# LuizGuzzo/Monocular_Depth_Estimation

Hardware: AMD Instinct MI355X
Metric: training images/sec at 640x480 bs=32/GPU (GuideDepth, SSIM+0.1*L1, Adam) (higher is better)
Workload: dtype fp32; 1 GPU; GuideDepth (DDRNet-23-slim + 3 guided upsampling blocks) train step, BASELINE cfg2, BN in train mode; global_batch=32, per_gpu_batch=32, resolution=640x480, parallelism=dp1

## Files before the change

### include/mde_abi.h

```cpp
#ifndef MDE_ABI_H
#define MDE_ABI_H

#include <stddef.h>
#include <stdint.h>

#ifdef __cplusplus
extern "C" {
#endif

#define MDE_ABI_VERSION 1

#define MDE_F32 0
#define MDE_BF16 1

#define MDE_OK 0
#define MDE_ERR_INVALID_ARG (-1)
#define MDE_ERR_UNSUPPORTED (-2)

int mde_abi_version(void);
const char* mde_status_string(int status);


int mde_bilinear_fwd(const void* x, void* y, int64_t n, int64_t c, int64_t hi,
                     int64_t wi, int64_t ho, int64_t wo, float scale_h,
                     float scale_w, int align_corners, int dtype, void* stream);
int mde_bilinear_bwd(const void* gy, void* gx, int64_t n, int64_t c,
                     int64_t hi, int64_t wi, int64_t ho, int64_t wo,
                     float scale_h, float scale_w, int align_corners,
                     int dtype, void* stream);
int mde_bilinear_bwd2_supported(int64_t n, int64_t c, int64_t hi, int64_t wi, int64_t ho,
                                int64_t wo, float scale_h, float scale_w, int align_corners);
int mde_bilinear_bwd2(const void* gy, const void* gy2, void* gx, int64_t n, int64_t c,
                      int64_t hi, int64_t wi, int64_t ho, int64_t wo, float scale_h,
                      float scale_w, int align_corners, int dtype, void* stream);

int mde_nearest_fwd(const void* x, void* y, int64_t n, int64_t c, int64_t hi,
                    int64_t wi, int64_t ho, int64_t wo, float scale_h,
                    float scale_w, int dtype, void* stream);
int mde_nearest_bwd(const void* gy, void* gx, int64_t n, int64_t c, int64_t hi,
                    int64_t wi, int64_t ho, int64_t wo, float scale_h,
                    float scale_w, int dtype, void* stream);
int mde_nearest_pyramid_supported(int64_t n, int64_t c, int64_t h, int64_t w);
int mde_nearest_pyramid(const void* x, void* half, void* quarter, int64_t n, int64_t c, int64_t h,
                        int64_t w, int dtype, void* stream);

size_t mde_se_workspace(int64_t n, int64_t c, int64_t cr, int64_t h,
                        int64_t w);
int mde_se_fwd(const void* xa, int64_t ca, const void* xb, int64_t cb,
               const float* w1, const float* w2, int64_t cr, void* out,
               float* s, float* hidden, float* mean, int64_t n, int64_t h,
               int64_t w, void* workspace, int dtype, void* stream);
int mde_se_bwd(const void* gout, const void* xa, int64_t ca, const void* xb,
               int64_t cb, const float* w1, const float* w2, int64_t cr,
               const float* s, const float* hidden, const float* mean,
               void* gxa, void* gxb, float* gw1, float* gw2, int64_t n,
               int64_t h, int64_t w, void* workspace, int dtype, void* stream);
int mde_se_gate_fwd(const void* xa, int64_t ca, const void* xb, int64_t cb,
                    const float* w1, const float* b1, const float* w2, const float* b2,
                    int64_t cr, int gate, void* out, float* s, float* hidden, float* mean,
                    int64_t n, int64_t h, int64_t w, void* workspace, int dtype,
                    void* stream);
int mde_se_gate_bwd(const void* gout, const void* xa, int64_t ca, const void* xb,
                    int64_t cb, const float* w1, const float* w2, const float* b2,
                    int64_t cr, int gate, const float* s, const float* hidden,
                    const float* mean, void* gxa, void* gxb, float* gw1, float* gb1,
                    float* gw2, float* gb2, int64_t n, int64_t h, int64_t w,
                    void* workspace, int dtype, void* stream);
size_t mde_se_bn_workspace(int64_t n, int64_t c, int64_t cr, int64_t h, int64_t w);
int mde_se_bn_fwd(const void* ya, int64_t ca, const void* yb, int64_t cb, const float* scale,
                  const float* shift, const float* w1, const float* w2, int64_t cr, void* out,
                  float* s, float* hidden, float* mean, int64_t n, int64_t h, int64_t w,
                  void* workspace, int dtype, void* stream);
int mde_se_bn_bwd(const void* gout, const void* ya, int64_t ca, const void* yb, int64_t cb,
                  const float* scale, const float* shift, const float* bn_mean,
                  const float* bn_invstd, int training, const float* w1, const float* w2,
                  int64_t cr, const float* s, const float* hidden, const float* mean, void* gya,
                  void* gyb, float* ggamma, float* gbeta, float* gw1, float* gw2, int64_t n,
                  int64_t h, int64_t w, void* workspace, int dtype, void* stream);

int mde_skip_reduce_fwd(const void* r, const void* d, const float* wt,
                        const float* b, void* out, int64_t n, int64_t cin,
                        int64_t cout, int64_t h, int64_t w, int dtype,
                        void* stream);
size_t mde_skip_reduce_workspace(int64_t n, int64_t cin, int64_t cout,
                                 int64_t h, int64_t w);
int mde_skip_reduce_bwd(const void* gout, const void* r, const void* d,
                        const float* wt, void* gs, float* gw, float* gb,
                        int64_t n, int64_t cin, int64_t cout, int64_t h,
                        int64_t w, void* workspace, int dtype, void* stream);
int mde_skip_reduce_bn_supported(int64_t cin, int64_t cout, int64_t h, int64_t w, int sums);
size_t mde_skip_reduce_bn_workspace(int64_t n, int64_t cin, int64_t cout, int64_t h, int64_t w);
int mde_skip_reduce_bn_fwd(const void* r, const void* d, const float* in_scale,
                           const float* in_shift, const float* wt, const float* b, void* out,
                           int64_t n, int64_t cin, int64_t cout, int64_t h, int64_t w, int dtype,
                           void* stream);
int mde_skip_reduce_bn_bwd(const void* gout, const void* r, const void* d, const float* in_scale,
                           const float* in_shift, const float* in_mean, const float* wt, void* gs,
                           float* gw, float* gb, float* in_sums, int64_t n, int64_t cin,
                           int64_t cout, int64_t h, int64_t w, void* workspace, int dtype,
                           void* stream);

size_t mde_minmax_workspace(int64_t numel);
int mde_minmax(const void* x, int64_t numel, float* minmax, void* workspace,
               int dtype, void* stream);
int mde_depthnorm_apply(const void* x, const float* minmax, void* y,
                        int64_t numel, int dtype, void* stream);

size_t mde_ssim3_l1_workspace(int64_t b, int64_t h, int64_t w);
int mde_ssim3_l1_fwd(const void* pred, const void* target,
                     const float* target_minmax, float w_ssim, float w_l1,
                     float* loss, void* grad_pred, void* grad_target,
                     int64_t b, int64_t h, int64_t w, void* workspace,
                     int dtype, void* stream);

size_t mde_depth_loss_workspace(int64_t b, int64_t h, int64_t w);
int mde_depth_loss_fwd(const void* pred, const void* gt, float alpha,
                       float beta, float gamma, float max_depth, float* out,
                       int64_t b, int64_t h, int64_t w, void* workspace,
                       int dtype, void* stream);
int mde_depth_loss_bwd(const void* pred, const void* gt, float alpha,
                       float beta, float gamma, float max_depth,
                       const float* fwd_out, const float* gout,
                       void* grad_pred, int64_t b, int64_t h, int64_t w,
                       void* workspace, int dtype, void* stream);

size_t mde_batchnorm_workspace(int64_t n, int64_t c, int64_t h, int64_t w);
int mde_batchnorm_fwd_train(const void* x, const float* gamma, const float* beta,
                            const float* prebias, float* running_mean,
                            float* running_var, int64_t* num_batches_tracked,
                            float momentum, float eps, const void* residual,
                            void* y, float* save_mean, float* save_invstd,
                            int64_t n, int64_t c, int64_t h, int64_t w, int act,
                            void* workspace, int dtype, void* stream);
int mde_batchnorm_fwd_eval(const void* x, const float* gamma, const float* beta,
                           const float* prebias, const float* running_mean,
                           const float* running_var, float eps,
                           const void* residual, void* y, float* save_mean,
                           float* save_invstd, int64_t n, int64_t c, int64_t h,
                           int64_t w, int act, int dtype, void* stream);
int mde_batchnorm_fwd_coef(const void* x, const float* gamma, const float* beta,
                           const float* prebias, float* running_mean, float* running_var,
                           int64_t* num_batches_tracked, float momentum, float eps,
                           int training, float* scale, float* shift, float* save_mean,
                           float* save_invstd, int64_t n, int64_t c, int64_t h, int64_t w,
                           void* workspace, int dtype, void* stream);
int mde_batchnorm_bwd(const void* gy, const void* x, const void* residual,
                      const float* gamma, const float* beta, const float* mean,
                      const float* invstd, int training, void* gx,
                      void* gresidual, float* ggamma, float* gbeta,
                      float* gprebias, int64_t n, int64_t c, int64_t h,
                      int64_t w, int act, void* workspace, int dtype,
                      void* stream);
int mde_batchnorm_fwd_train_stats(const void* x, const float* gamma, const float* beta,
                                  const float* prebias, float* running_mean, float* running_var,
                                  int64_t* num_batches_tracked, float momentum, float eps,
                                  const void* residual, void* y, float* save_mean,
                                  float* save_invstd, int64_t n, int64_t c, int64_t h, int64_t w,
                                  int act, const float* stats, int64_t stats_blocks,
                                  void* workspace, int dtype, void* stream);
int mde_batchnorm_fwd_coef_stats(const void* x, const float* gamma, const float* beta,
                                 const float* prebias, float* running_mean, float* running_var,
                                 int64_t* num_batches_tracked, float momentum, float eps,
                                 float* scale, float* shift, float* save_mean, float* save_invstd,
                                 int64_t n, int64_t c, int64_t h, int64_t w, const float* stats,
                                 int64_t stats_blocks, void* workspace, int dtype, void* stream);
int mde_batchnorm_bwd_apply(const void* gy, const void* x, const void* residual,
                            const float* gamma, const float* beta, const float* mean,
                            const float* invstd, int training, const float* sums, void* gx,
                            void* gresidual, float* ggamma, float* gbeta, float* gprebias,
                            int64_t n, int64_t c, int64_t h, int64_t w, int act, int dtype,
                            void* stream);

size_t mde_window_attn_workspace(int64_t b, int64_t h, int64_t w, int64_t c,
                                 int64_t heads, int64_t window);
int mde_window_attn_fwd(const void* qk, const float* qk_bias, const void* v,
                        const float* v_bias, const float* table, void* out, int64_t b,
                        int64_t h, int64_t w, int64_t c, int64_t heads, int64_t window,
                        int64_t shift, int dtype, void* stream);
int mde_window_attn_bwd(const void* gout, const void* qk, const float* qk_bias,
                        const void* v, const float* v_bias, const float* table, void* gqk,
                        void* gv, float* gtable, float* gqk_bias, float* gv_bias, int64_t b,
                        int64_t h, int64_t w, int64_t c, int64_t heads, int64_t window,
                        int64_t shift, void* workspace, int dtype, void* stream);

size_t mde_colsum_workspace(int64_t t_rows, int64_t n);
int mde_colsum(const void* g, float* gb, int64_t t_rows, int64_t n, void* workspace, int dtype,
               void* stream);
int mde_gelu_bwd_colsum(const void* dh, const void* a, void* da, float* gb, int64_t t_rows,
                        int64_t n, void* workspace, int dtype, void* stream);

size_t mde_linear_wgrad_workspace(int64_t t_rows, int64_t m, int64_t n);
int mde_linear_wgrad(const void* g, const void* x, float* gw, float* gb, int64_t t_rows,
                     int64_t m, int64_t n, void* workspace, int dtype, void* stream);

size_t mde_chansum_workspace(int64_t n, int64_t c, int64_t hw);
int mde_chansum(const void* g, float* gb, int64_t n, int64_t c, int64_t hw, void* workspace,
                int dtype, void* stream);

int mde_head_conv_supported(int64_t n, int64_t c, int64_t h, int64_t w);
int mde_head_conv_fwd(const void* x, const float* weight, const float* bias, void* y, int64_t n,
                      int64_t c, int64_t h, int64_t w, int dtype, void* stream);
int mde_head_conv_dgrad(const void* gy, const float* weight, void* gx, int64_t n, int64_t c,
                        int64_t h, int64_t w, int dtype, void* stream);
size_t mde_head_conv_wgrad_workspace(int64_t n, int64_t c, int64_t h, int64_t w);
int mde_head_conv_wgrad(const void* gy, const void* x, float* gweight, int64_t n, int64_t c,
                        int64_t h, int64_t w, void* workspace, int dtype, void* stream);

int mde_pointwise_supported(int64_t cin, int64_t cout, int64_t h, int64_t w);
size_t mde_pointwise_workspace(int64_t n, int64_t cin, int64_t cout, int64_t h, int64_t w);
int mde_pointwise_fwd(const void* x, const float* in_scale, const float* in_shift,
                      const float* weight, void* y, int64_t n, int64_t cin, int64_t cout,
                      int64_t h, int64_t w, int dtype, void* stream);
int mde_pointwise_bwd(const void* gy, const void* x, const float* in_scale,
                      const float* in_shift, const float* weight, void* gx, float* gweight,
                      int64_t n, int64_t cin, int64_t cout, int64_t h, int64_t w,
                      void* workspace, int dtype, void* stream);
int mde_pointwise_stats_blocks(int64_t n, int64_t cin, int64_t cout, int64_t h, int64_t w);
int mde_pointwise_fwd_stats(const void* x, const float* in_scale, const float* in_shift,
                            const float* weight, void* y, float* stats, int64_t n, int64_t cin,
                            int64_t cout, int64_t h, int64_t w, int dtype, void* stream);
int mde_pointwise_bwd_bn(const void* gy, const void* x, const float* in_scale,
                         const float* in_shift, const float* in_mean, const float* weight,
                         void* gx, float* gweight, float* in_sums, int64_t n, int64_t cin,
                         int64_t cout, int64_t h, int64_t w, void* workspace, int dtype,
                         void* stream);

int mde_conv3x3_supported(int64_t cin, int64_t cout, int pass, int dtype);
int mde_conv3x3_fwd(const void* x, const float* weight, void* y, int64_t n, int64_t cin,
                    int64_t cout, int64_t h, int64_t w, int dtype, void* stream);
int mde_conv3x3_stats_blocks(int64_t n, int64_t cin, int64_t cout, int64_t h, int64_t w,
                             int dtype);
int mde_conv3x3_fwd_stats(const void* x, const float* weight, void* y, float* stats, int64_t n,
                          int64_t cin, int64_t cout, int64_t h, int64_t w, int dtype,
                          void* stream);
int mde_conv3x3_bwd_data(const void* gy, const float* weight, void* gx, int64_t n,
                         int64_t cin, int64_t cout, int64_t h, int64_t w, int dtype,
                         void* stream);
size_t mde_conv3x3_wgrad_workspace(int64_t n, int64_t cin, int64_t cout, int64_t h, int64_t w,
                                   int dtype);
int mde_conv3x3_wgrad(const void* gy, const void* x, float* gweight, int64_t n, int64_t cin,
                      int64_t cout, int64_t h, int64_t w, void* workspace, int dtype,
                      void* stream);

int mde_conv3x3s2_supported(int64_t cin, int64_t cout, int dtype);
size_t mde_conv3x3s2_wgrad_workspace(int64_t n, int64_t cin, int64_t cout, int64_t h, int64_t w,
                                     int dtype);
int mde_conv3x3s2_wgrad(const void* gy, const void* x, float* gweight, int64_t n, int64_t cin,
                        int64_t cout, int64_t h, int64_t w, void* workspace, int dtype,
                        void* stream);

size_t mde_dwconv_workspace(int64_t n, int64_t c, int64_t h, int64_t w, int64_t k,
                            int64_t stride, int64_t pad);
int mde_dwconv_fwd(const void* x, const float* weight, void* y, int64_t n, int64_t c,
                   int64_t h, int64_t w, int64_t k, int64_t stride, int64_t pad, int dtype,
                   void* stream);
int mde_dwconv_bwd(const void* gy, const void* x, const float* weight, void* gx,
                   float* gweight, int64_t n, int64_t c, int64_t h, int64_t w, int64_t k,
                   int64_t stride, int64_t pad, void* workspace, int dtype, void* stream);

size_t mde_layernorm_workspace(int64_t rows, int64_t c);
int mde_layernorm_fwd(const void* x, const float* gamma, const float* beta, void* y,
                      float* mean, float* rstd, int64_t rows, int64_t c, float eps, int dtype,
                      void* stream);
int mde_layernorm_bwd(const void* gy, const void* x, const float* gamma, const float* mean,
                      const float* rstd, void* gx, float* ggamma, float* gbeta, int64_t rows,
                      int64_t c, void* workspace, int dtype, void* stream);
int mde_layernorm_add_fwd(const void* x, const void* r, const float* gamma, const float* beta,
                          void* sum, void* y, float* mean, float* rstd, int64_t rows, int64_t c,
                          float eps, int dtype, void* stream);
int mde_layernorm_bwd_res(const void* gy, const void* x, const void* gres, const float* gamma,
                          const float* mean, const float* rstd, void* gx, float* ggamma,
                          float* gbeta, int64_t rows, int64_t c, void* workspace, int dtype,
                          void* stream);

int mde_transpose(const void* x, void* y, int64_t batch, int64_t m, int64_t n, int dtype,
                  void* stream);

int mde_nyu_augment(const void* image, const void* depth, const int32_t* flags, float* image_out,
                    float* depth_out, int64_t n, int64_t h, int64_t w, int64_t dh, int64_t dw,
                    int depth_bits, void* stream);

size_t mde_eval_workspace(int64_t n, int64_t h, int64_t w);
int mde_eval_sums(const void* pred, const void* gt, int64_t n, int64_t h, int64_t w,
                  float min_depth, float max_depth, int mode, const int32_t* crop,
                  void* workspace, double* sums, int dtype, void* stream);

int mde_conv3x3_guide_bf16_stats_blocks(int64_t n, int64_t cout, int64_t h, int64_t w);
int mde_conv3x3_guide_bf16_fwd(const float* x, const float* weight, void* y, float* stats,
                               int64_t n, int64_t cout, int64_t h, int64_t w, void* stream);

int mde_conv1x1_supported(int64_t cin, int64_t cout, int64_t h, int64_t w, int stride,
                          int dtype);
int mde_conv1x1_fwd(const void* x, const float* weight, void* y, int64_t n, int64_t cin,
                    int64_t cout, int64_t h, int64_t w, int stride, int dtype, void* stream);
int mde_conv1x1_bwd_data(const void* gy, const float* weight, void* gx, int64_t n, int64_t cin,
                         int64_t cout, int64_t h, int64_t w, int stride, int dtype,
                         void* stream);
size_t mde_conv1x1_wgrad_workspace(int64_t n, int64_t cin, int64_t cout, int64_t h, int64_t w,
                                   int stride, int dtype);
int mde_conv1x1_wgrad(const void* gy, const void* x, float* gweight, int64_t n, int64_t cin,
                      int64_t cout, int64_t h, int64_t w, int stride, void* workspace, int dtype,
                      void* stream);

int mde_conv3x3s2_fwd_supported(int64_t cin, int64_t cout, int64_t h, int64_t w, int dtype);
int mde_conv3x3s2_dgrad_supported(int64_t cin, int64_t cout, int64_t h, int64_t w, int dtype);
int mde_conv3x3s2_fwd(const void* x, const float* weight, void* y, int64_t n, int64_t cin,
                      int64_t cout, int64_t h, int64_t w, int dtype, void* stream);
int mde_conv3x3s2_bwd_data(const void* gy, const float* weight, void* gx, int64_t n, int64_t cin,
// ... 93 lines not shown
```

### monocular_depth_estimation_amd/_abi.py

```python
from __future__ import annotations

import ctypes
import os

import torch

LIB_PATH = os.environ.get("MDE_HIP_LIB") or os.path.join(
    os.path.dirname(os.path.abspath(__file__)), "libmde_hip.so")

MDE_F32 = 0
MDE_BF16 = 1

_c = ctypes
_vp = _c.c_void_p
_i64 = _c.c_int64
_f32 = _c.c_float
_int = _c.c_int
_sz = _c.c_size_t
_fp = _c.POINTER(_c.c_float)

SIGNATURES = {
    "mde_abi_version": (_int, []),
    "mde_status_string": (_c.c_char_p, [_int]),
    "mde_bilinear_fwd": (_int, [_vp, _vp, _i64, _i64, _i64, _i64, _i64, _i64, _f32, _f32, _int, _int, _vp]),
    "mde_bilinear_bwd": (_int, [_vp, _vp, _i64, _i64, _i64, _i64, _i64, _i64, _f32, _f32, _int, _int, _vp]),
    "mde_bilinear_bwd2_supported": (_int, [_i64, _i64, _i64, _i64, _i64, _i64, _f32, _f32, _int]),
    "mde_bilinear_bwd2": (_int, [_vp, _vp, _vp, _i64, _i64, _i64, _i64, _i64, _i64, _f32, _f32, _int,
                                 _int, _vp]),
    "mde_nearest_fwd": (_int, [_vp, _vp, _i64, _i64, _i64, _i64, _i64, _i64, _f32, _f32, _int, _vp]),
    "mde_nearest_bwd": (_int, [_vp, _vp, _i64, _i64, _i64, _i64, _i64, _i64, _f32, _f32, _int, _vp]),
    "mde_nearest_pyramid_supported": (_int, [_i64, _i64, _i64, _i64]),
    "mde_nearest_pyramid": (_int, [_vp, _vp, _vp, _i64, _i64, _i64, _i64, _int, _vp]),
    "mde_se_workspace": (_sz, [_i64, _i64, _i64, _i64, _i64]),
    "mde_se_fwd": (_int, [_vp, _i64, _vp, _i64, _vp, _vp, _i64, _vp, _vp, _vp, _vp,
                          _i64, _i64, _i64, _vp, _int, _vp]),
    "mde_se_bwd": (_int, [_vp, _vp, _i64, _vp, _i64, _vp, _vp, _i64, _vp, _vp, _vp,
                          _vp, _vp, _vp, _vp, _i64, _i64, _i64, _vp, _int, _vp]),
    "mde_se_bn_workspace": (_sz, [_i64, _i64, _i64, _i64, _i64]),
    "mde_se_bn_fwd": (_int, [_vp, _i64, _vp, _i64, _vp, _vp, _vp, _vp, _i64, _vp, _vp, _vp, _vp,
                             _i64, _i64, _i64, _vp, _int, _vp]),
    "mde_se_bn_bwd": (_int, [_vp, _vp, _i64, _vp, _i64, _vp, _vp, _vp, _vp, _int, _vp, _vp, _i64,
                             _vp, _vp, _vp, _vp, _vp, _vp, _vp, _vp, _vp, _i64, _i64, _i64, _vp,
                             _int, _vp]),
    "mde_skip_reduce_fwd": (_int, [_vp, _vp, _vp, _vp, _vp, _i64, _i64, _i64, _i64, _i64, _int, _vp]),
    "mde_skip_reduce_workspace": (_sz, [_i64, _i64, _i64, _i64, _i64]),
    "mde_skip_reduce_bwd": (_int, [_vp, _vp, _vp, _vp, _vp, _vp, _vp, _i64, _i64, _i64, _i64, _i64,
                                   _vp, _int, _vp]),
    "mde_skip_reduce_bn_supported": (_int, [_i64, _i64, _i64, _i64, _int]),
    "mde_skip_reduce_bn_workspace": (_sz, [_i64, _i64, _i64, _i64, _i64]),
    "mde_skip_reduce_bn_fwd": (_int, [_vp, _vp, _vp, _vp, _vp, _vp, _vp, _i64, _i64, _i64, _i64, _i64,
                                      _int, _vp]),
    "mde_skip_reduce_bn_bwd": (_int, [_vp, _vp, _vp, _vp, _vp, _vp, _vp, _vp, _vp, _vp, _vp, _i64,
                                      _i64, _i64, _i64, _i64, _vp, _int, _vp]),
    "mde_minmax_workspace": (_sz, [_i64]),
    "mde_minmax": (_int, [_vp, _i64, _vp, _vp, _int, _vp]),
    "mde_depthnorm_apply": (_int, [_vp, _vp, _vp, _i64, _int, _vp]),
    "mde_ssim3_l1_workspace": (_sz, [_i64, _i64, _i64]),
    "mde_ssim3_l1_fwd": (_int, [_vp, _vp, _vp, _f32, _f32, _vp, _vp, _vp, _i64, _i64, _i64, _vp, _int, _vp]),
    "mde_depth_loss_workspace": (_sz, [_i64, _i64, _i64]),
    "mde_depth_loss_fwd": (_int, [_vp, _vp, _f32, _f32, _f32, _f32, _vp, _i64, _i64, _i64, _vp, _int, _vp]),
    "mde_depth_loss_bwd": (_int, [_vp, _vp, _f32, _f32, _f32, _f32, _vp, _vp, _vp, _i64, _i64, _i64,
                                  _vp, _int, _vp]),
    "mde_batchnorm_workspace": (_sz, [_i64, _i64, _i64, _i64]),
    "mde_batchnorm_fwd_train": (_int, [_vp, _vp, _vp, _vp, _vp, _vp, _vp, _f32, _f32, _vp, _vp, _vp,
                                       _vp, _i64, _i64, _i64, _i64, _int, _vp, _int, _vp]),
    "mde_batchnorm_fwd_eval": (_int, [_vp, _vp, _vp, _vp, _vp, _vp, _f32, _vp, _vp, _vp, _vp,
                                      _i64, _i64, _i64, _i64, _int, _int, _vp]),
    "mde_batchnorm_bwd": (_int, [_vp, _vp, _vp, _vp, _vp, _vp, _vp, _int, _vp, _vp, _vp, _vp, _vp,
                                 _i64, _i64, _i64, _i64, _int, _vp, _int, _vp]),
    "mde_batchnorm_bwd_apply": (_int, [_vp, _vp, _vp, _vp, _vp, _vp, _vp, _int, _vp, _vp, _vp, _vp,
                                       _vp, _vp, _i64, _i64, _i64, _i64, _int, _int, _vp]),
    "mde_window_attn_workspace": (_sz, [_i64, _i64, _i64, _i64, _i64, _i64]),
    "mde_window_attn_fwd": (_int, [_vp, _vp, _vp, _vp, _vp, _vp, _i64, _i64, _i64, _i64, _i64, _i64,
                                   _i64, _int, _vp]),
    "mde_window_attn_bwd": (_int, [_vp, _vp, _vp, _vp, _vp, _vp, _vp, _vp, _vp, _vp, _vp, _i64, _i64,
                                   _i64, _i64, _i64, _i64, _i64, _vp, _int, _vp]),
    "mde_se_gate_fwd": (_int, [_vp, _i64, _vp, _i64, _vp, _vp, _vp, _vp, _i64, _int, _vp, _vp, _vp,
                               _vp, _i64, _i64, _i64, _vp, _int, _vp]),
    "mde_se_gate_bwd": (_int, [_vp, _vp, _i64, _vp, _i64, _vp, _vp, _vp, _i64, _int, _vp, _vp, _vp,
                               _vp, _vp, _vp, _vp, _vp, _vp, _i64, _i64, _i64, _vp, _int, _vp]),
    "mde_pointwise_supported": (_int, [_i64, _i64, _i64, _i64]),
    "mde_pointwise_workspace": (_sz, [_i64, _i64, _i64, _i64, _i64]),
    "mde_pointwise_fwd": (_int, [_vp, _vp, _vp, _vp, _vp, _i64, _i64, _i64, _i64, _i64, _int, _vp]),
    "mde_pointwise_bwd": (_int, [_vp, _vp, _vp, _vp, _vp, _vp, _vp, _i64, _i64, _i64, _i64, _i64,
                                 _vp, _int, _vp]),
    "mde_pointwise_stats_blocks": (_int, [_i64, _i64, _i64, _i64, _i64]),
    "mde_pointwise_fwd_stats": (_int, [_vp, _vp, _vp, _vp, _vp, _vp, _i64, _i64, _i64, _i64, _i64,
                                       _int, _vp]),
    "mde_conv3x3_stats_blocks": (_int, [_i64, _i64, _i64, _i64, _i64, _int]),
    "mde_conv3x3_fwd_stats": (_int, [_vp, _vp, _vp, _vp, _i64, _i64, _i64, _i64, _i64, _int, _vp]),
    "mde_batchnorm_fwd_train_stats": (_int, [_vp, _vp, _vp, _vp, _vp, _vp, _vp, _f32, _f32, _vp,
                                             _vp, _vp, _vp, _i64, _i64, _i64, _i64, _int, _vp,
                                             _i64, _vp, _int, _vp]),
    "mde_batchnorm_fwd_coef_stats": (_int, [_vp, _vp, _vp, _vp, _vp, _vp, _vp, _f32, _f32, _vp,
                                            _vp, _vp, _vp, _i64, _i64, _i64, _i64, _vp, _i64, _vp,
                                            _int, _vp]),
    "mde_pointwise_bwd_bn": (_int, [_vp, _vp, _vp, _vp, _vp, _vp, _vp, _vp, _vp, _i64, _i64, _i64,
                                    _i64, _i64, _vp, _int, _vp]),
    "mde_batchnorm_fwd_coef": (_int, [_vp, _vp, _vp, _vp, _vp, _vp, _vp, _f32, _f32, _int, _vp, _vp,
                                      _vp, _vp, _i64, _i64, _i64, _i64, _vp, _int, _vp]),
    "mde_conv3x3_supported": (_int, [_i64, _i64, _int, _int]),
    "mde_conv3x3_fwd": (_int, [_vp, _vp, _vp, _i64, _i64, _i64, _i64, _i64, _int, _vp]),
    "mde_conv3x3_bwd_data": (_int, [_vp, _vp, _vp, _i64, _i64, _i64, _i64, _i64, _int, _vp]),
    "mde_conv3x3_wgrad_workspace": (_sz, [_i64, _i64, _i64, _i64, _i64, _int]),
    "mde_conv3x3_wgrad": (_int, [_vp, _vp, _vp, _i64, _i64, _i64, _i64, _i64, _vp, _int, _vp]),
    "mde_conv3x3s2_supported": (_int, [_i64, _i64, _int]),
    "mde_conv3x3s2_wgrad_workspace": (_sz, [_i64, _i64, _i64, _i64, _i64, _int]),
    "mde_conv3x3s2_wgrad": (_int, [_vp, _vp, _vp, _i64, _i64, _i64, _i64, _i64, _vp, _int, _vp]),
    "mde_dwconv_workspace": (_sz, [_i64, _i64, _i64, _i64, _i64, _i64, _i64]),
    "mde_dwconv_fwd": (_int, [_vp, _vp, _vp, _i64, _i64, _i64, _i64, _i64, _i64, _i64, _int, _vp]),
    "mde_dwconv_bwd": (_int, [_vp, _vp, _vp, _vp, _vp, _i64, _i64, _i64, _i64, _i64, _i64, _i64,
                              _vp, _int, _vp]),
    "mde_layernorm_workspace": (_sz, [_i64, _i64]),
    "mde_layernorm_fwd": (_int, [_vp, _vp, _vp, _vp, _vp, _vp, _i64, _i64, _f32, _int, _vp]),
    "mde_layernorm_bwd": (_int, [_vp, _vp, _vp, _vp, _vp, _vp, _vp, _vp, _i64, _i64, _vp, _int,
                                 _vp]),
    "mde_layernorm_add_fwd": (_int, [_vp, _vp, _vp, _vp, _vp, _vp, _vp, _vp, _i64, _i64, _f32,
                                      _int, _vp]),
    "mde_layernorm_bwd_res": (_int, [_vp, _vp, _vp, _vp, _vp, _vp, _vp, _vp, _vp, _i64, _i64,
                                      _vp, _int, _vp]),
    "mde_transpose": (_int, [_vp, _vp, _i64, _i64, _i64, _int, _vp]),
    "mde_nyu_augment": (_int, [_vp, _vp, _vp, _vp, _vp, _i64, _i64, _i64, _i64, _i64, _int, _vp]),
    "mde_eval_workspace": (_sz, [_i64, _i64, _i64]),
    "mde_eval_sums": (_int, [_vp, _vp, _i64, _i64, _i64, _f32, _f32, _int, _c.POINTER(_c.c_int32), _vp,
                             _vp, _int, _vp]),
    "mde_colsum_workspace": (_sz, [_i64, _i64]),
    "mde_colsum": (_int, [_vp, _vp, _i64, _i64, _vp, _int, _vp]),
    "mde_head_conv_supported": (_int, [_i64, _i64, _i64, _i64]),
    "mde_head_conv_fwd": (_int, [_vp, _vp, _vp, _vp, _i64, _i64, _i64, _i64, _int, _vp]),
    "mde_head_conv_dgrad": (_int, [_vp, _vp, _vp, _i64, _i64, _i64, _i64, _int, _vp]),
    "mde_head_conv_wgrad_workspace": (_sz, [_i64, _i64, _i64, _i64]),
    "mde_head_conv_wgrad": (_int, [_vp, _vp, _vp, _i64, _i64, _i64, _i64, _vp, _int, _vp]),
    "mde_chansum_workspace": (_sz, [_i64, _i64, _i64]),
    "mde_chansum": (_int, [_vp, _vp, _i64, _i64, _i64, _vp, _int, _vp]),
    "mde_linear_wgrad_workspace": (_sz, [_i64, _i64, _i64]),
    "mde_linear_wgrad": (_int, [_vp, _vp, _vp, _vp, _i64, _i64, _i64, _vp, _int, _vp]),
    "mde_gelu_bwd_colsum": (_int, [_vp, _vp, _vp, _vp, _i64, _i64, _vp, _int, _vp]),
    "mde_conv1x1_supported": (_int, [_i64, _i64, _i64, _i64, _int, _int]),
    "mde_conv1x1_fwd": (_int, [_vp, _vp, _vp, _i64, _i64, _i64, _i64, _i64, _int, _int, _vp]),
    "mde_conv1x1_bwd_data": (_int, [_vp, _vp, _vp, _i64, _i64, _i64, _i64, _i64, _int, _int, _vp]),
    "mde_conv1x1_wgrad_workspace": (_sz, [_i64, _i64, _i64, _i64, _i64, _int, _int]),
    "mde_conv1x1_wgrad": (_int, [_vp, _vp, _vp, _i64, _i64, _i64, _i64, _i64, _int, _vp, _int,
                                 _vp]),
    "mde_conv3x3s2_fwd_supported": (_int, [_i64, _i64, _i64, _i64, _int]),
    "mde_conv3x3s2_dgrad_supported": (_int, [_i64, _i64, _i64, _i64, _int]),
    "mde_conv3x3s2_fwd": (_int, [_vp, _vp, _vp, _i64, _i64, _i64, _i64, _i64, _int, _vp]),
    "mde_conv3x3s2_bwd_data": (_int, [_vp, _vp, _vp, _i64, _i64, _i64, _i64, _i64, _int, _vp]),
    "mde_conv3x3_wide_supported": (_int, [_i64, _i64, _i64, _i64, _int, _int]),
    "mde_conv3x3_wide_fwd": (_int, [_vp, _vp, _vp, _i64, _i64, _i64, _i64, _i64, _int, _vp]),
    "mde_conv3x3_wide_bwd_data": (_int, [_vp, _vp, _vp, _i64, _i64, _i64, _i64, _i64, _int, _vp]),
    "mde_wino_mode": (_int, [_int]),
    "mde_wino_supported": (_int, [_i64, _i64, _i64, _i64, _int]),
    "mde_wino_weight_bytes": (_sz, [_i64, _i64]),
    "mde_wino_weight": (_int, [_vp, _vp, _i64, _i64, _int, _vp]),
    "mde_wino_weight2": (_int, [_vp, _vp, _vp, _i64, _i64, _vp]),
    "mde_wino_weight_blocks": (_i64, [_i64, _i64, _int]),
    "mde_wino_weight_table": (_int, [_vp, _int, _i64, _i64, _vp]),
    "mde_wino_conv": (_int, [_vp, _vp, _vp, _i64, _i64, _i64, _i64, _i64, _int, _int, _vp]),
    "mde_wino_conv_acc": (_int, [_vp, _vp, _vp, _vp, _i64, _i64, _i64, _i64, _i64, _int, _int, _vp]),
    "mde_wino_conv_stats": (_int, [_vp, _vp, _vp, _vp, _i64, _i64, _i64, _i64, _i64, _int, _int,
                                   _vp]),
    "mde_wino_stats_blocks": (_int, [_i64, _i64, _i64, _i64, _i64]),
    "mde_batchnorm_stats_route": (_int, [_i64, _i64, _i64, _i64, _i64, _int]),
    "mde_bn_chan_mode": (_int, [_int]),
    "mde_convbf_supported": (_int, [_i64, _i64, _i64, _i64, _int, _int, _int]),
    "mde_convbf_supported_n": (_int, [_i64, _i64, _i64, _i64, _i64, _int, _int, _int]),
    "mde_convbf_flops": (_c.c_double, [_i64, _i64, _i64, _i64, _i64, _int, _int, _int]),
    "mde_stem_bf16_supported": (_int, [_i64, _i64, _i64, _i64]),
    "mde_stem_bf16_fwd": (_int, [_vp, _vp, _vp, _i64, _i64, _i64, _i64, _vp]),
    "mde_stem_bf16_wgrad_workspace": (_sz, [_i64, _i64, _i64, _i64]),
    "mde_stem_bf16_wgrad": (_int, [_vp, _vp, _vp, _i64, _i64, _i64, _i64, _vp, _vp]),
    "mde_conv3x3_guide_bf16_wgrad_workspace": (_sz, [_i64, _i64, _i64, _i64]),
    "mde_conv3x3_guide_bf16_wgrad": (_int, [_vp, _vp, _vp, _i64, _i64, _i64, _i64, _vp, _vp]),
    "mde_convbf_pack_elems": (_sz, [_i64, _i64, _int, _int]),
    "mde_convbf_pack": (_int, [_vp, _vp, _i64, _i64, _int, _int, _vp]),
    "mde_convbf_pack_both": (_int, [_vp, _vp, _vp, _i64, _i64, _int, _vp]),
    "mde_convbf_pack_table": (_int, [_vp, _int, _i64, _i64, _vp]),
    "mde_convbf_stats_blocks": (_int, [_i64, _i64, _i64, _i64, _i64, _int, _int]),
    "mde_convbf_fwd": (_int, [_vp, _vp, _vp, _vp, _i64, _i64, _i64, _i64, _i64, _int, _int, _vp]),
    "mde_convbf_bwd_data": (_int, [_vp, _vp, _vp, _i64, _i64, _i64, _i64, _i64, _int, _int, _vp]),
    "mde_convbf_wgrad_workspace": (_sz, [_i64, _i64, _i64, _i64, _i64, _int, _int]),
# ... 160 lines not shown
```

### monocular_depth_estimation_amd/csrc/bn.hip

```cpp
#include <cmath>

#include <cstdlib>
#include <type_traits>

#include "common.h"

namespace {

constexpr int kTarget = 2048;
constexpr int kMinSlice = 4096;
constexpr int kPlaneChunk4 = 1024;
constexpr int64_t kMaxApplyRecords = 256;

struct Geo {
  int64_t c, hw, total;
  int slices;
  int64_t slice_len;
};

int64_t env_or(const char* name, int64_t dflt) {
  const char* v = std::getenv(name);
  return v && *v ? std::atoll(v) : dflt;
}

// ... 359 lines not shown
      };
      const float4 z4 = make_float4(0.f, 0.f, 0.f, 0.f);
      for (; i + (kRedDepth - 1) * kStep < i1; i += kRedDepth * kStep) {
        float4 g[kRedDepth], v[kRedDepth], q[kRedDepth];
#pragma unroll
        for (int k = 0; k < kRedDepth; ++k) {
          const int64_t off = base + cur.off;
          g[k] = ld4(gy + off);
          v[k] = ld4(x + off);
          q[k] = r ? ld4(r + off) : z4;
          cur.advance(kStep, hw, chw);
        }
#pragma unroll
        for (int k = 0; k < kRedDepth; ++k) acc(g[k], v[k], q[k]);
      }
      for (; i < i1; i += kStep) {
        const int64_t off = base + cur.off;
        acc(ld4(gy + off), ld4(x + off), r ? ld4(r + off) : z4);
        cur.advance(kStep, hw, chw);
      }
    }
  } else {
    for (int64_t i = i0 + threadIdx.x; i < i1; i += 256) {
      const int64_t nn = i / hw, p = i - nn * hw;
      const int64_t off = base + nn * chw + p;
      const float v = ld1(x + off);
      const float a = dy_eff(ld1(gy + off), v, r ? ld1(r + off) : 0.f, sc, sh, act);
      s1 += a;
      s2 += a * (v - mu);
    }
  }
  const float t1 = mde::block_sum256(s1, red);
  const float t2 = mde::block_sum256(s2, red);
  if (threadIdx.x == 0) {
    float* o = part + (ch * slices + s) * 2;
    o[0] = t1;
    o[1] = t2;
  }
}

struct BwdArgs {
  const float* gamma;
  const float* beta;
  const float* mean;
  const float* invstd;
  const float* part;
  int slices;
  int64_t total;
  int training;
  float* ggamma;
  float* gbeta;
  float* gprebias;
};

struct BwdCh {
  float sc, sh, A, B, D;
};

__device__ BwdCh bwd_channel(const BwdArgs& P, int64_t ch, double sdy,
                             double sdyx, bool owner) {
  BwdCh r;
  const double is = (double)P.invstd[ch];
  const double mu = (double)P.mean[ch];
  const double scale = (double)P.gamma[ch] * is;
  double A = scale, B = 0.0, D = 0.0;
  const double n = (double)P.total;
  if (P.training) {
    B = -scale * is * is * sdyx / n;
    D = -scale * sdy / n - B * mu;
  }
  if (owner) {
    if (P.ggamma) P.ggamma[ch] = (float)(sdyx * is);
    if (P.gbeta) P.gbeta[ch] = (float)sdy;
    if (P.gprebias) P.gprebias[ch] = (float)(A * sdy + B * n * mu + D * n);
  }
  r.sc = P.gamma[ch] * P.invstd[ch];
  r.sh = P.beta[ch] - P.mean[ch] * r.sc;
  r.A = (float)A;
  r.B = (float)B;
  r.D = (float)D;
  return r;
}

template <typename T>
__global__ void __launch_bounds__(256)
    bn_bwd_apply_plane_kernel(const T* __restrict__ gy, const T* __restrict__ x,
                              const T* __restrict__ r, T* __restrict__ gx,
                              T* __restrict__ gr, int64_t c, int64_t hw, int act,
                              BwdArgs P) {
  __shared__ float cf[5];
  const int64_t plane = blockIdx.y;
  const int64_t ch = plane % c;
  const int64_t hw4 = hw >> 2;
  const T* gp = gy + plane * hw;
  const T* xp = x + plane * hw;
  const T* rp = r ? r + plane * hw : nullptr;
  T* op = gx + plane * hw;
  T* orp = gr ? gr + plane * hw : nullptr;
  const int64_t b0 = blockIdx.x * (int64_t)kPlaneChunk4;
  constexpr int KK = kPlaneChunk4 / 256;
  float4 g4[KK], v4[KK], q4[KK];
#pragma unroll
  for (int k = 0; k < KK; ++k) {
    const int64_t i = b0 + k * 256 + threadIdx.x;
    const int64_t ic = i < hw4 ? i : hw4 - 1;
    g4[k] = ld4_nt(gp + 4 * ic);
    v4[k] = ld4_nt(xp + 4 * ic);
    q4[k] = rp ? ld4_nt(rp + 4 * ic) : make_float4(0.f, 0.f, 0.f, 0.f);
  }
  if (threadIdx.x < 64) {
    double a, b;
    wave_slices(P.part, ch, P.slices, &a, &b);
    if (threadIdx.x == 0) {
      const BwdCh k = bwd_channel(P, ch, a, b, blockIdx.x == 0 && plane < c);
      cf[0] = k.sc; cf[1] = k.sh; cf[2] = k.A; cf[3] = k.B; cf[4] = k.D;
    }
  }
  __syncthreads();
  const float sc = cf[0], sh = cf[1], A = cf[2], B = cf[3], D = cf[4];
#pragma unroll
  for (int k = 0; k < KK; ++k) {
    const int64_t i = b0 + k * 256 + threadIdx.x;
    if (i < hw4) {
      const float4 g = g4[k], v = v4[k], q = q4[k];
      const float4 e = make_float4(dy_eff(g.x, v.x, q.x, sc, sh, act),
                                   dy_eff(g.y, v.y, q.y, sc, sh, act),
                                   dy_eff(g.z, v.z, q.z, sc, sh, act),
                                   dy_eff(g.w, v.w, q.w, sc, sh, act));
      st4_nt(op + 4 * i, make_float4(A * e.x + B * v.x + D, A * e.y + B * v.y + D,
                                     A * e.z + B * v.z + D, A * e.w + B * v.w + D));
      if (orp) st4_nt(orp + 4 * i, e);
    }
  }
}

template <typename T>
__global__ void __launch_bounds__(256)
    bn_bwd_apply_table_kernel(const T* __restrict__ gy, const T* __restrict__ x,
                              const T* __restrict__ r, T* __restrict__ gx,
                              T* __restrict__ gr, int64_t planes, int64_t c,
                              int64_t hw, int act, BwdArgs P) {
  extern __shared__ float tab[];
  const PlaneShare ps(planes, c);
  for (int64_t kk = threadIdx.x; kk < ps.nch; kk += blockDim.x) {
    const int64_t ch = ps.channel(kk, c);
    double a = 0.0, b = 0.0;
    for (int s = 0; s < P.slices; ++s) {
      a += (double)P.part[(ch * P.slices + s) * 2];
      b += (double)P.part[(ch * P.slices + s) * 2 + 1];
    }
    const BwdCh k = bwd_channel(P, ch, a, b, ps.owner(ch));
    tab[ch] = k.sc;
    tab[c + ch] = k.sh;
    tab[2 * c + ch] = k.A;
    tab[3 * c + ch] = k.B;
    tab[4 * c + ch] = k.D;
  }
  __syncthreads();
  const int64_t total = planes * hw;
  if (table_vec(total, hw)) {
    const uint32_t hw4 = (uint32_t)(hw >> 2), cc = (uint32_t)c;
    const uint32_t t1 = (uint32_t)(ps.p1 * (hw >> 2));
    for (uint32_t t = (uint32_t)(ps.p0 * (hw >> 2)) + threadIdx.x; t < t1; t += blockDim.x) {
      const uint32_t ch = (t / hw4) % cc;
      const int64_t o = 4 * (int64_t)t;
      const float sc = tab[ch], sh = tab[c + ch];
// ... 512 lines not shown
  if (!dtype_ok(dtype)) return MDE_ERR_UNSUPPORTED;
  if (!x || !gamma || !beta || !y || !save_mean || !save_invstd || !workspace || !stats ||
      stats_blocks <= 0 || stats_blocks > 0x7fffffff || (!running_mean != !running_var) ||
      act < 0 || act > 2 || !args_ok(n, c, h, w))
    return MDE_ERR_INVALID_ARG;
  hipStream_t s = (hipStream_t)stream;
  const int64_t hw = h * w;
  if (dtype == MDE_BF16 ? chan_mode<bf16>(n, hw) : chan_mode<float>(n, hw))
    return mde_batchnorm_fwd_train(x, gamma, beta, prebias, running_mean, running_var,
                                   num_batches_tracked, momentum, eps, residual, y, save_mean,
                                   save_invstd, n, c, h, w, act, workspace, dtype, stream);
  float* part = (float*)workspace;
  if (plane_mode(hw) && stats_blocks <= kMaxApplyRecords) {
    FwdArgs A{gamma, beta, prebias, part, 0, n * hw, hw, eps, momentum, running_mean,
              running_var, num_batches_tracked, save_mean, save_invstd, 1, stats,
              (int)stats_blocks};
    if (dtype == MDE_BF16)
      return launch_fwd_apply((const bf16*)x, (const bf16*)residual, (bf16*)y, n, c, hw, act, A, s);
    return launch_fwd_apply((const float*)x, (const float*)residual, (float*)y, n, c, hw, act, A, s);
  }
  const double mb = 16.0 * (double)c * stats_blocks;
  if (dtype == MDE_BF16)
    MDE_LAUNCH(mde::K_BN_FINAL, mb, s, (bn_stats_merge_kernel<bf16, false>), dim3((unsigned)c),
               dim3(256), 0, (const bf16*)x, stats, (int)stats_blocks, hw, part, FwdArgs{},
               nullptr, nullptr);
  else
    MDE_LAUNCH(mde::K_BN_FINAL, mb, s, (bn_stats_merge_kernel<float, false>), dim3((unsigned)c),
               dim3(256), 0, (const float*)x, stats, (int)stats_blocks, hw, part, FwdArgs{},
               nullptr, nullptr);
  FwdArgs A{gamma, beta, prebias, part, 1, n * hw, hw, eps, momentum,
            running_mean, running_var, num_batches_tracked, save_mean, save_invstd, 1};
  if (dtype == MDE_BF16)
    return launch_fwd_apply((const bf16*)x, (const bf16*)residual, (bf16*)y, n, c, hw, act, A, s);
  return launch_fwd_apply((const float*)x, (const float*)residual, (float*)y, n, c, hw, act, A, s);
}

int mde_batchnorm_fwd_coef_stats(const void* x, const float* gamma, const float* beta,
                                 const float* prebias, float* running_mean, float* running_var,
                                 int64_t* num_batches_tracked, float momentum, float eps,
                                 float* scale, float* shift, float* save_mean, float* save_invstd,
                                 int64_t n, int64_t c, int64_t h, int64_t w, const float* stats,
                                 int64_t stats_blocks, void* workspace, int dtype, void* stream) {
  if (!dtype_ok(dtype)) return MDE_ERR_UNSUPPORTED;
  if (!x || !gamma || !beta || !scale || !shift || !save_mean || !save_invstd || !workspace ||
      !stats || stats_blocks <= 0 || stats_blocks > 0x7fffffff ||
      (!running_mean != !running_var) || !args_ok(n, c, h, w))
    return MDE_ERR_INVALID_ARG;
  hipStream_t s = (hipStream_t)stream;
  const int64_t hw = h * w;
  float* part = (float*)workspace;
  const double mb = 16.0 * (double)c * stats_blocks;
  FwdArgs A{gamma, beta, prebias, part, 1, n * hw, hw, eps, momentum, running_mean, running_var,
            num_batches_tracked, save_mean, save_invstd, 1};
  if (dtype == MDE_BF16) {
    MDE_LAUNCH(mde::K_BN_FINAL, mb + 8.0 * (double)c, s, (bn_stats_merge_kernel<bf16, true>),
               dim3((unsigned)c), dim3(256), 0, (const bf16*)x, stats, (int)stats_blocks, hw,
               part, A, scale, shift);
  } else {
    MDE_LAUNCH(mde::K_BN_FINAL, mb + 8.0 * (double)c, s, (bn_stats_merge_kernel<float, true>),
               dim3((unsigned)c), dim3(256), 0, (const float*)x, stats, (int)stats_blocks, hw,
               part, A, scale, shift);
  }
  return MDE_OK;
}

int mde_batchnorm_bwd_apply(const void* gy, const void* x, const void* residual,
                            const float* gamma, const float* beta, const float* mean,
                            const float* invstd, int training, const float* sums, void* gx,
                            void* gresidual, float* ggamma, float* gbeta, float* gprebias,
                            int64_t n, int64_t c, int64_t h, int64_t w, int act, int dtype,
                            void* stream) {
  if (!dtype_ok(dtype)) return MDE_ERR_UNSUPPORTED;
  if (!gy || !x || !gamma || !beta || !mean || !invstd || !sums || !gx || act < 0 || act > 2 ||
      !args_ok(n, c, h, w) || (gresidual && !residual && act))
    return MDE_ERR_INVALID_ARG;
  hipStream_t s = (hipStream_t)stream;
  const int64_t hw = h * w;
  BwdArgs P{gamma, beta, mean, invstd, sums, 1, n * hw, training, ggamma, gbeta, gprebias};
  return dtype == MDE_BF16
             ? bwd_apply<bf16>(gy, x, residual, gx, gresidual, n, c, hw, act, P, s)
             : bwd_apply<float>(gy, x, residual, gx, gresidual, n, c, hw, act, P, s);
}

}
```

### monocular_depth_estimation_amd/csrc/se.hip

```cpp
#include "common.h"

namespace {

constexpr int kChunk = 16384;

template <typename T>
__device__ __forceinline__ const T* plane_ptr(const T* xa, int64_t ca, const T* xb, int64_t cb,
                                              int64_t nidx, int64_t ch, int64_t hw) {
  return ch < ca ? xa + (nidx * ca + ch) * hw
                 : xb + (nidx * cb + (ch - ca)) * hw;
}

enum { kSum = 0, kDot = 1, kBnRelu = 2 };

__device__ __forceinline__ float bnrelu(float v, float sc, float sh) {
  return fmaxf(fmaf(v, sc, sh), 0.f);
}

template <int MODE, typename T = float>
__global__ void __launch_bounds__(256)
    se_partial_kernel(const T* __restrict__ g, const T* __restrict__ xa,
                      int64_t ca, const T* __restrict__ xb, int64_t cb,
                      int64_t hw, int chunks, float* __restrict__ part,
                      const float* __restrict__ scale = nullptr,
// ... 248 lines not shown
      const int64_t nidx = plane / c, ch = plane % c;
      float* dst = ch < ca ? (gxa ? gxa + (nidx * ca + ch) * hw : nullptr)
                           : (gxb ? gxb + (nidx * cb + ch - ca) * hw : nullptr);
      if (!dst) continue;
      const float sc = s[plane], add = dm[plane] * inv_hw;
      const float4 q = *reinterpret_cast<const float4*>(g + plane * hw + i);
      *reinterpret_cast<float4*>(dst + i) =
          make_float4(q.x * sc + add, q.y * sc + add, q.z * sc + add,
                      q.w * sc + add);
    }
  } else {
    const int64_t total = planes * hw;
    for (int64_t t = blockIdx.x * (int64_t)blockDim.x + threadIdx.x; t < total;
         t += (int64_t)gridDim.x * blockDim.x) {
      const int64_t plane = t / hw, i = t - plane * hw;
      const int64_t nidx = plane / c, ch = plane % c;
      float* dst = ch < ca ? (gxa ? gxa + (nidx * ca + ch) * hw : nullptr)
                           : (gxb ? gxb + (nidx * cb + ch - ca) * hw : nullptr);
      if (dst) dst[i] = g[t] * s[plane] + dm[plane] * inv_hw;
    }
  }
}

template <typename T = float>
__global__ void __launch_bounds__(256)
    sebn_bwd_reduce_kernel(const T* __restrict__ g, const T* __restrict__ ya, int64_t ca,
                           const T* __restrict__ yb, int64_t cb, int64_t hw, int chunks,
                           const float* __restrict__ scale, const float* __restrict__ shift,
                           const float* __restrict__ mean, float* __restrict__ part_e,
                           float* __restrict__ part4) {
  __shared__ float red[4];
  const int64_t c = ca + cb;
  const int64_t plane = blockIdx.y;
  const int64_t nidx = plane / c, ch = plane % c;
  const T* y = plane_ptr(ya, ca, yb, cb, nidx, ch, hw);
  const T* gp = g + plane * hw;
  const float sc = scale[ch], sh = shift[ch], mu = mean[ch];
  const int64_t beg = (int64_t)blockIdx.x * kChunk;
  const int64_t end = beg + kChunk < hw ? beg + kChunk : hw;
  float A = 0.f, B = 0.f, C = 0.f, D = 0.f, E = 0.f;
  auto one = [&](float yv, float gv) {
    const float z = fmaf(yv, sc, sh);
    if (z > 0.f) {
      const float d = yv - mu;
      A += gv;
      B += 1.f;
      C += gv * d;
      D += d;
      E += gv * z;
    }
  };
  if ((hw & 3) == 0) {
    for (int64_t i = beg + 4 * threadIdx.x; i < end; i += 4 * 256) {
      const float4 v = mde::ld4(y + i);
      const float4 q = mde::ld4(gp + i);
      one(v.x, q.x); one(v.y, q.y); one(v.z, q.z); one(v.w, q.w);
    }
  } else {
    for (int64_t i = beg + threadIdx.x; i < end; i += 256) one(mde::ld1(y + i), mde::ld1(gp + i));
  }
  A = mde::block_sum256(A, red);
  B = mde::block_sum256(B, red);
  C = mde::block_sum256(C, red);
  D = mde::block_sum256(D, red);
  E = mde::block_sum256(E, red);
  if (threadIdx.x == 0) {
    const int64_t k = plane * chunks + blockIdx.x;
    part_e[k] = E;
    float* o = part4 + 4 * k;
    o[0] = A; o[1] = B; o[2] = C; o[3] = D;
  }
}

constexpr int kMaxSeN = 256;

__global__ void __launch_bounds__(256)
    sebn_bwd_combine_kernel(const float* __restrict__ part4, int chunks, int64_t n, int64_t c,
                            int64_t hw, const float* __restrict__ s, float* __restrict__ dm,
                            const float* __restrict__ scale, const float* __restrict__ invstd,
                            int training, float* __restrict__ ggamma, float* __restrict__ gbeta,
                            float* __restrict__ coef, int cr, const float* __restrict__ w1,
                            const float* __restrict__ dz, const float* __restrict__ dh,
                            const float* __restrict__ hidden, const float* __restrict__ mean,
                            float* __restrict__ gw1, float* __restrict__ gw2) {
  __shared__ double red[2][4];
  __shared__ float dms[kMaxSeN];
  if ((int64_t)blockIdx.x >= c) {
    se_wgrad_body((int64_t)(blockIdx.x - c) * blockDim.x + threadIdx.x, (int)n, (int)c, cr, dz, dh,
                  hidden, mean, gw1, gw2, nullptr, nullptr);
    return;
  }
  const int64_t ch = blockIdx.x;
  const double inv_hw = 1.0 / (double)hw;
  double s1 = 0.0, s2 = 0.0;
  for (int64_t n0 = 0; n0 < n; n0 += kMaxSeN) {
    const int64_t nb = n - n0 < kMaxSeN ? n - n0 : kMaxSeN;
    if (n0 > 0) __syncthreads();
    {
      const int lane = threadIdx.x & 63, wid = threadIdx.x >> 6;
      for (int64_t k = wid; k < nb; k += 4) {
        const int64_t nn = n0 + k;
        float acc = 0.f;
        for (int j = lane; j < cr; j += 64) acc += w1[(int64_t)j * c + ch] * dh[nn * cr + j];
        acc = mde::wave_sum(acc);
        if (lane == 0) {
          dms[k] = acc;
          dm[nn * c + ch] = acc;
        }
      }
    }
    __syncthreads();
    for (int64_t i = threadIdx.x; i < nb * chunks; i += 256) {
      const int64_t plane = (n0 + i / chunks) * c + ch;
      const float* p = part4 + 4 * (plane * chunks + i % chunks);
      const double sv = s[plane], q = (double)dms[i / chunks] * inv_hw;
      s1 += sv * (double)p[0] + q * (double)p[1];
      s2 += sv * (double)p[2] + q * (double)p[3];
    }
  }
#pragma unroll
  for (int o = 32; o > 0; o >>= 1) {
    s1 += __shfl_xor(s1, o, 64);
    s2 += __shfl_xor(s2, o, 64);
  }
  const int lane = threadIdx.x & 63, wid = threadIdx.x >> 6;
  if (lane == 0) {
    red[0][wid] = s1;
    red[1][wid] = s2;
  }
  __syncthreads();
  if (threadIdx.x != 0) return;
  s1 = (red[0][0] + red[0][1]) + (red[0][2] + red[0][3]);
  s2 = (red[1][0] + red[1][1]) + (red[1][2] + red[1][3]);
  const double is = invstd[ch], sc = scale[ch], cnt = (double)n * (double)hw;
  if (ggamma) ggamma[ch] = (float)(is * s2);
  if (gbeta) gbeta[ch] = (float)s1;
  coef[2 * ch] = training ? (float)(-sc * s1 / cnt) : 0.f;
  coef[2 * ch + 1] = training ? (float)(-sc * is * is * s2 / cnt) : 0.f;
}

template <typename T = float>
__global__ void __launch_bounds__(256)
    sebn_bwd_apply_kernel(const T* __restrict__ g, const T* __restrict__ ya, int64_t ca,
                          const T* __restrict__ yb, int64_t cb, int64_t hw, int64_t planes,
                          const float* __restrict__ s, const float* __restrict__ dm, float inv_hw,
                          const float* __restrict__ scale, const float* __restrict__ shift,
                          const float* __restrict__ mean, const float* __restrict__ coef,
                          T* __restrict__ gya, T* __restrict__ gyb) {
  const int64_t c = ca + cb;
  auto one = [](float yv, float gv, float sc, float sh, float P, float Q, float R, float Tc,
                float mu) {
    const float z = fmaf(yv, sc, sh);
    return (z > 0.f ? fmaf(P, gv, Q) : 0.f) + fmaf(Tc, yv - mu, R);
  };
  if ((hw & 3) == 0) {
    const int64_t hw4 = hw >> 2;
    const int64_t total = planes * hw4;
    for (int64_t t = blockIdx.x * (int64_t)blockDim.x + threadIdx.x; t < total;
         t += (int64_t)gridDim.x * blockDim.x) {
      const int64_t plane = t / hw4, i = (t - plane * hw4) << 2;
      const int64_t nidx = plane / c, ch = plane % c;
      const T* y = plane_ptr(ya, ca, yb, cb, nidx, ch, hw);
      T* dst = ch < ca ? gya + (nidx * ca + ch) * hw : gyb + (nidx * cb + ch - ca) * hw;
      const float sc = scale[ch], sh = shift[ch], mu = mean[ch];
      const float P = sc * s[plane], Q = sc * dm[plane] * inv_hw;
      const float R = coef[2 * ch], Tc = coef[2 * ch + 1];
      const float4 v = mde::ld4(y + i);
      const float4 q = mde::ld4(g + plane * hw + i);
      mde::st4(dst + i, make_float4(one(v.x, q.x, sc, sh, P, Q, R, Tc, mu),
                                    one(v.y, q.y, sc, sh, P, Q, R, Tc, mu),
                                    one(v.z, q.z, sc, sh, P, Q, R, Tc, mu),
                                    one(v.w, q.w, sc, sh, P, Q, R, Tc, mu)));
    }
  } else {
    const int64_t total = planes * hw;
    for (int64_t t = blockIdx.x * (int64_t)blockDim.x + threadIdx.x; t < total;
         t += (int64_t)gridDim.x * blockDim.x) {
      const int64_t plane = t / hw, i = t - plane * hw;
      const int64_t nidx = plane / c, ch = plane % c;
      const T* y = plane_ptr(ya, ca, yb, cb, nidx, ch, hw);
      T* dst = ch < ca ? gya + (nidx * ca + ch) * hw : gyb + (nidx * cb + ch - ca) * hw;
      const float sc = scale[ch];
      mde::st1(dst + i, one(mde::ld1(y + i), mde::ld1(g + t), sc, shift[ch], sc * s[plane],
                            sc * dm[plane] * inv_hw, coef[2 * ch], coef[2 * ch + 1], mean[ch]));
    }
  }
}

inline int stream_grid(int64_t work) {
  const int64_t b = mde::cdiv(work, 256);
  return (int)(b < 1 ? 1 : (b > 8192 ? 8192 : b));
}

struct SeWs;
int se_bfc(const SeWs& ws, int chunks, int64_t n, int64_t c, int64_t cr, const float* w1,
           const float* w2, const float* b2, int gate, const float* s, const float* hidden,
           const float* mean, float* gw1, float* gw2, float* gb1, float* gb2, hipStream_t st,
           bool tail = false);

struct SeWs {
  float* part;
  float* dz;
  float* dh;
  float* dm;
  float* part4;
  float* coef;
};

inline int64_t se_chunks(int64_t hw) { return mde::cdiv(hw, kChunk); }

inline size_t round16(size_t b) { return (b + 15) & ~size_t(15); }

SeWs se_carve(void* ws, int64_t n, int64_t c, int64_t cr, int64_t hw) {
  char* p = (char*)ws;
  SeWs r;
  r.part = (float*)p;
  p += round16(sizeof(float) * n * c * se_chunks(hw));
  r.dz = (float*)p;
  p += round16(sizeof(float) * n * c);
  r.dh = (float*)p;
  p += round16(sizeof(float) * n * cr);
// ... 79 lines not shown
                    void* workspace, int dtype, void* stream) {
  if (dtype != MDE_F32) return MDE_ERR_UNSUPPORTED;
  const int64_t c = ca + cb, hw = h * w;
  if (gate < 0 || gate > 1) return MDE_ERR_INVALID_ARG;
  if (!gout || !xa || ca <= 0 || cb < 0 || (cb > 0 && !xb) || !w1 || !w2 ||
      cr <= 0 || !s || !hidden || !mean || !gw1 || !gw2 || n <= 0 ||
      hw <= 0 || !workspace || c > 4096 || cr > 4096 || n > 65535)
    return MDE_ERR_INVALID_ARG;
  hipStream_t st = (hipStream_t)stream;
  SeWs ws = se_carve(workspace, n, c, cr, hw);
  const int chunks = (int)se_chunks(hw);
  const double big = 4.0 * n * c * (double)hw;
  MDE_LAUNCH(mde::K_SE_BWD_DOT, 2.0 * big, st, (se_partial_kernel<kDot, float>),
             dim3(chunks, (unsigned)(n * c)), dim3(256), 0,
             (const float*)gout, (const float*)xa, ca, (const float*)xb, cb,
             hw, chunks, ws.part);
  const int fcs = se_bfc(ws, chunks, n, c, cr, w1, w2, b2, gate, s, hidden, mean, gw1, gw2, gb1,
                         gb2, st);
  if (fcs) return fcs;
  if (gxa || gxb) {
    MDE_LAUNCH(mde::K_SE_BWD_APPLY, 2.0 * big, st, se_apply_kernel,
               dim3(stream_grid(n * c * hw / 4)), dim3(256), 0,
               (const float*)gout, ca, cb, hw, n * c, s, ws.dm,
               1.f / (float)hw, (float*)gxa, (float*)gxb);
  }
  return MDE_OK;
}

int mde_se_fwd(const void* xa, int64_t ca, const void* xb, int64_t cb,
               const float* w1, const float* w2, int64_t cr, void* out,
               float* s, float* hidden, float* mean, int64_t n, int64_t h,
               int64_t w, void* workspace, int dtype, void* stream) {
  return mde_se_gate_fwd(xa, ca, xb, cb, w1, nullptr, w2, nullptr, cr, 0, out, s, hidden,
                         mean, n, h, w, workspace, dtype, stream);
}

int mde_se_bwd(const void* gout, const void* xa, int64_t ca, const void* xb,
               int64_t cb, const float* w1, const float* w2, int64_t cr,
               const float* s, const float* hidden, const float* mean,
               void* gxa, void* gxb, float* gw1, float* gw2, int64_t n,
               int64_t h, int64_t w, void* workspace, int dtype, void* stream) {
  return mde_se_gate_bwd(gout, xa, ca, xb, cb, w1, w2, nullptr, cr, 0, s, hidden, mean, gxa,
                         gxb, gw1, nullptr, gw2, nullptr, n, h, w, workspace, dtype, stream);
}

size_t mde_se_bn_workspace(int64_t n, int64_t c, int64_t cr, int64_t h, int64_t w) {
  return mde_se_workspace(n, c, cr, h, w) + round16(sizeof(float) * 4 * n * c * se_chunks(h * w)) +
         round16(sizeof(float) * 2 * c);
}

}

template <typename T>
static int se_bn_fwd_t(const void* ya, int64_t ca, const void* yb, int64_t cb, const float* scale,
                       const float* shift, const float* w1, const float* w2, int64_t cr, void* out,
                       float* s, float* hidden, float* mean, int64_t n, int64_t hw,
                       void* workspace, hipStream_t st) {
  const int64_t c = ca + cb;
  SeWs ws = se_carve(workspace, n, c, cr, hw);
  const int chunks = (int)se_chunks(hw);
  const double big = (double)sizeof(T) * n * c * (double)hw;
  MDE_LAUNCH(mde::K_SE_SQUEEZE, big, st, (se_partial_kernel<kBnRelu, T>),
             dim3(chunks, (unsigned)(n * c)), dim3(256), 0, nullptr, (const T*)ya, ca,
             (const T*)yb, cb, hw, chunks, ws.part, scale, shift);
  MDE_LAUNCH(mde::K_SE_FC, 4.0 * (c * cr + 2.0 * n * c), st, se_fc1_kernel,
             dim3((unsigned)n, (unsigned)mde::cdiv(cr, kOutPerBlock)), dim3(1024),
             sizeof(float) * c, ws.part, chunks, (int)c, (int)cr, 1.f / (float)hw, w1, nullptr,
             hidden, mean);
  MDE_LAUNCH(mde::K_SE_FC, 4.0 * (c * cr + 2.0 * n * c), st, se_fc2_kernel,
             dim3((unsigned)n, (unsigned)mde::cdiv(c, kOutPerBlock)), dim3(1024),
             sizeof(float) * cr, (int)c, (int)cr, w2, nullptr, 0, hidden, s);
  MDE_LAUNCH(mde::K_SE_SCALE, 2.0 * big, st, (se_scale_kernel<true, T>),
             dim3(stream_grid(n * c * hw / 4)), dim3(256), 0, (const T*)ya, ca, (const T*)yb, cb,
             hw, n * c, s, (T*)out, scale, shift);
  return MDE_OK;
}

template <typename T>
static int se_bn_bwd_t(const void* gout, const void* ya, int64_t ca, const void* yb, int64_t cb,
                       const float* scale, const float* shift, const float* bn_mean,
                       const float* bn_invstd, int training, const float* w1, const float* w2,
                       int64_t cr, const float* s, const float* hidden, const float* mean,
                       void* gya, void* gyb, float* ggamma, float* gbeta, float* gw1, float* gw2,
                       int64_t n, int64_t hw, void* workspace, hipStream_t st) {
  const int64_t c = ca + cb;
  SeWs ws = se_carve(workspace, n, c, cr, hw);
  const int chunks = (int)se_chunks(hw);
  const double big = (double)sizeof(T) * n * c * (double)hw;
  MDE_LAUNCH(mde::K_SE_BWD_DOT, 2.0 * big, st, sebn_bwd_reduce_kernel<T>,
             dim3(chunks, (unsigned)(n * c)), dim3(256), 0, (const T*)gout, (const T*)ya, ca,
             (const T*)yb, cb, hw, chunks, scale, shift, bn_mean, ws.part, ws.part4);
  const int fcs = se_bfc(ws, chunks, n, c, cr, w1, w2, nullptr, 0, s, hidden, mean, gw1, gw2,
                         nullptr, nullptr, st, true);
  if (fcs) return fcs;
  MDE_LAUNCH(mde::K_SE_BWD_FC, 16.0 * n * c * chunks + 4.0 * (3.0 * c * cr + n * (3.0 * c + 3.0 * cr)),
             st, sebn_bwd_combine_kernel,
             dim3((unsigned)(c + mde::cdiv(2 * c * cr, 256))), dim3(256), 0, ws.part4, chunks, n, c,
             hw, s, ws.dm, scale, bn_invstd, training, ggamma, gbeta, ws.coef, (int)cr, w1, ws.dz,
             ws.dh, hidden, mean, gw1, gw2);
  MDE_LAUNCH(mde::K_SE_BWD_APPLY, 3.0 * big, st, sebn_bwd_apply_kernel<T>,
             dim3(stream_grid(n * c * hw / 4)), dim3(256), 0, (const T*)gout, (const T*)ya, ca,
             (const T*)yb, cb, hw, n * c, s, ws.dm, 1.f / (float)hw, scale, shift, bn_mean,
             ws.coef, (T*)gya, (T*)gyb);
  return MDE_OK;
}

extern "C" {

int mde_se_bn_fwd(const void* ya, int64_t ca, const void* yb, int64_t cb, const float* scale,
                  const float* shift, const float* w1, const float* w2, int64_t cr, void* out,
                  float* s, float* hidden, float* mean, int64_t n, int64_t h, int64_t w,
                  void* workspace, int dtype, void* stream) {
  if (dtype != MDE_F32 && dtype != MDE_BF16) return MDE_ERR_UNSUPPORTED;
  const int64_t c = ca + cb, hw = h * w;
  if (!ya || ca <= 0 || cb < 0 || (cb > 0 && !yb) || !scale || !shift || !w1 || !w2 ||
      cr <= 0 || !out || !s || !hidden || !mean || n <= 0 || hw <= 0 || !workspace ||
      c > 4096 || cr > 4096 || n > 65535 || n * c > 65535)
    return MDE_ERR_INVALID_ARG;
  hipStream_t st = (hipStream_t)stream;
  return dtype == MDE_BF16
             ? se_bn_fwd_t<mde::bf16>(ya, ca, yb, cb, scale, shift, w1, w2, cr, out, s, hidden,
                                      mean, n, hw, workspace, st)
             : se_bn_fwd_t<float>(ya, ca, yb, cb, scale, shift, w1, w2, cr, out, s, hidden, mean,
                                  n, hw, workspace, st);
}

int mde_se_bn_bwd(const void* gout, const void* ya, int64_t ca, const void* yb, int64_t cb,
                  const float* scale, const float* shift, const float* bn_mean,
                  const float* bn_invstd, int training, const float* w1, const float* w2,
                  int64_t cr, const float* s, const float* hidden, const float* mean, void* gya,
                  void* gyb, float* ggamma, float* gbeta, float* gw1, float* gw2, int64_t n,
                  int64_t h, int64_t w, void* workspace, int dtype, void* stream) {
  if (dtype != MDE_F32 && dtype != MDE_BF16) return MDE_ERR_UNSUPPORTED;
  const int64_t c = ca + cb, hw = h * w;
  if (!gout || !ya || ca <= 0 || cb < 0 || (cb > 0 && (!yb || !gyb)) || !gya || !scale ||
      !shift || !bn_mean || !bn_invstd || !w1 || !w2 || cr <= 0 || !s || !hidden || !mean ||
      !gw1 || !gw2 || n <= 0 || hw <= 0 || !workspace || c > 4096 || cr > 4096 ||
      n > 65535 || n * c > 65535)
    return MDE_ERR_INVALID_ARG;
  hipStream_t st = (hipStream_t)stream;
  return dtype == MDE_BF16
             ? se_bn_bwd_t<mde::bf16>(gout, ya, ca, yb, cb, scale, shift, bn_mean, bn_invstd,
                                      training, w1, w2, cr, s, hidden, mean, gya, gyb, ggamma,
                                      gbeta, gw1, gw2, n, hw, workspace, st)
             : se_bn_bwd_t<float>(gout, ya, ca, yb, cb, scale, shift, bn_mean, bn_invstd,
                                  training, w1, w2, cr, s, hidden, mean, gya, gyb, ggamma, gbeta,
                                  gw1, gw2, n, hw, workspace, st);
}

}
```

### monocular_depth_estimation_amd/csrc/skip.hip

```cpp
#include "common.h"

namespace {

constexpr int kMaxC = 64;

template <int CO, int PPT, bool BNR = false, typename T = float>
__global__ void __launch_bounds__(256)
    skip_fwd_kernel(const T* __restrict__ r, const T* __restrict__ d,
                    const float* __restrict__ wt, const float* __restrict__ b,
                    T* __restrict__ out, int64_t n, int cin, int cout,
                    int64_t hw, const float* __restrict__ isc = nullptr,
                    const float* __restrict__ ish = nullptr) {
  __shared__ float sw[kMaxC * kMaxC];
  __shared__ float sb[kMaxC];
  for (int i = threadIdx.x; i < cin * cout; i += blockDim.x) sw[i] = wt[i];
  for (int i = threadIdx.x; i < cout; i += blockDim.x) sb[i] = b[i];
  __syncthreads();
  const int64_t groups = hw / PPT;
  const int64_t total = n * groups;
  for (int64_t t = blockIdx.x * (int64_t)blockDim.x + threadIdx.x; t < total;
       t += (int64_t)gridDim.x * blockDim.x) {
    const int64_t nidx = t / groups;
    const int64_t p = (t - nidx * groups) * PPT;
    const T* rp = r + nidx * cin * hw + p;
// ... 169 lines not shown
                       const float* __restrict__ imean = nullptr) {
  static_assert(CI % 4 == 0 && (!BNS || BNR), "channel groups of 4; BN sums need BNR");
  constexpr int NG = CI / 4, QPB = 256 / NG;
  constexpr int ROW = CI + 1 + (BNS ? 2 * CI : 0);
  __shared__ float red[4][ROW];
  const int tid = threadIdx.x, grp = tid % NG, qi = tid / NG;
  float w[4], bs[4], bh[4], mu[4];
#pragma unroll
  for (int k = 0; k < 4; ++k) {
    const int c = 4 * grp + k;
    w[k] = wt[c];
    bs[k] = BNR ? isc[c] : 1.f;
    bh[k] = BNR ? ish[c] : 0.f;
    mu[k] = BNS ? imean[c] : 0.f;
  }
  float aw[4] = {}, e1[4] = {}, e2[4] = {}, ab = 0.f;
  const int64_t q4 = hw >> 2, total = n * q4;
  for (int64_t t = (int64_t)blockIdx.x * QPB + qi; t < total; t += (int64_t)gridDim.x * QPB) {
    const int64_t nidx = t / q4, p = (t - nidx * q4) << 2;
    const float4 gv = mde::ld4(g + nidx * hw + p);
    if (grp == 0) ab += (gv.x + gv.y) + (gv.z + gv.w);
    const int64_t base = (nidx * CI + 4 * grp) * hw + p;
    float4 a[4], e[4];
#pragma unroll
    for (int k = 0; k < 4; ++k) {
      a[k] = mde::ld4(r + base + k * hw);
      e[k] = mde::ld4(d + base + k * hw);
    }
#pragma unroll
    for (int k = 0; k < 4; ++k) {
      auto act = [&](float v) { return BNR ? fmaxf(v * bs[k] + bh[k], 0.f) : v; };
      const float4 sv = make_float4(act(a[k].x) + e[k].x, act(a[k].y) + e[k].y,
                                    act(a[k].z) + e[k].z, act(a[k].w) + e[k].w);
      aw[k] += (gv.x * sv.x + gv.y * sv.y) + (gv.z * sv.z + gv.w * sv.w);
      const float4 o4 = make_float4(w[k] * gv.x, w[k] * gv.y, w[k] * gv.z, w[k] * gv.w);
      mde::st4(gs + base + k * hw, o4);
      if constexpr (BNS) {
        const float av[4] = {a[k].x, a[k].y, a[k].z, a[k].w}, ov[4] = {o4.x, o4.y, o4.z, o4.w};
#pragma unroll
        for (int j = 0; j < 4; ++j) {
          const float ev = av[j] * bs[k] + bh[k] > 0.f ? ov[j] : 0.f;
          e1[k] += ev;
          e2[k] += ev * (av[j] - mu[k]);
        }
      }
    }
  }
  auto gsum = [&](float v) {
#pragma unroll
    for (int o = NG; o < 64; o <<= 1) v += __shfl_xor(v, o, 64);
    return v;
  };
  const int lane = tid & 63, wv = tid >> 6;
#pragma unroll
  for (int k = 0; k < 4; ++k) {
    const float sw = gsum(aw[k]);
    float s1 = 0.f, s2 = 0.f;
    if constexpr (BNS) {
      s1 = gsum(e1[k]);
      s2 = gsum(e2[k]);
    }
    if (lane < NG) {
      const int c = 4 * lane + k;
      red[wv][c] = sw;
      if constexpr (BNS) {
        red[wv][CI + 1 + 2 * c] = s1;
        red[wv][CI + 1 + 2 * c + 1] = s2;
      }
    }
  }
  const float sb = gsum(ab);
  if (lane == 0) red[wv][CI] = sb;
  __syncthreads();
  for (int i = tid; i < ROW; i += 256)
    slab[(int64_t)blockIdx.x * ROW + i] = (red[0][i] + red[1][i]) + (red[2][i] + red[3][i]);
}

using f4 = __attribute__((ext_vector_type(4))) float;

__device__ __forceinline__ f4 mfma4(float a, float b, f4 c) {
  return __builtin_amdgcn_mfma_f32_16x16x4f32(a, b, c, 0, 0, 0);
}

template <int CI, int CO, bool HAS_D, bool BNR = false, bool BNS = false, typename T = float>
__global__ void __launch_bounds__(256, CI * CO >= 4096 ? 1 : 2)
    skip_bwd_mfma_kernel(const T* __restrict__ g, const T* __restrict__ r,
                         const T* __restrict__ d, const float* __restrict__ wt,
                         T* __restrict__ gs, float* __restrict__ slab, int64_t n,
                         int64_t hw, const float* __restrict__ isc = nullptr,
                         const float* __restrict__ ish = nullptr,
                         const float* __restrict__ imean = nullptr) {
  constexpr int MT = CI / 16, OT = (CO + 15) / 16, KO = CO / 4;
  static_assert(CI % 16 == 0 && CO % 8 == 0, "tile shapes");
  static_assert(!BNS || (BNR && CI <= 32), "BN sums: fused BN-ReLU operand, cin <= 32");
  constexpr int ROW = CO * CI + CO + (BNS ? 2 * CI : 0);
  __shared__ float red[4][ROW];
  const int lane = threadIdx.x & 63, w = threadIdx.x >> 6, l16 = lane & 15, q4 = lane >> 4;
  float wa[MT][KO];
#pragma unroll
  for (int mt = 0; mt < MT; ++mt)
#pragma unroll
    for (int kk = 0; kk < KO; ++kk) wa[mt][kk] = wt[(4 * kk + q4) * CI + 16 * mt + l16];
  f4 gw[OT][MT];
#pragma unroll
  for (int ot = 0; ot < OT; ++ot)
#pragma unroll
    for (int mt = 0; mt < MT; ++mt) gw[ot][mt] = f4{0.f, 0.f, 0.f, 0.f};
  float gbp[OT] = {};
  float bsc[MT], bsh[MT];
#pragma unroll
  for (int mt = 0; mt < MT; ++mt) {
    bsc[mt] = BNR ? isc[16 * mt + l16] : 1.f;
    bsh[mt] = BNR ? ish[16 * mt + l16] : 0.f;
  }
  constexpr int SOFF = CO * CI + CO;
  float esc[BNS ? MT : 1][4], esh[BNS ? MT : 1][4], emu[BNS ? MT : 1][4];
  float es1[BNS ? MT : 1][4], es2[BNS ? MT : 1][4];
  if constexpr (BNS) {
#pragma unroll
    for (int mt = 0; mt < MT; ++mt)
#pragma unroll
      for (int i = 0; i < 4; ++i) {
        const int c = 16 * mt + 4 * q4 + i;
        esc[mt][i] = isc[c];
        esh[mt][i] = ish[c];
        emu[mt][i] = imean[c];
        es1[mt][i] = 0.f;
        es2[mt][i] = 0.f;
      }
  }
  const int64_t tpi = hw / 64;
  const int64_t tiles = n * tpi;
  for (int64_t t = (int64_t)blockIdx.x * 4 + w; t < tiles; t += (int64_t)gridDim.x * 4) {
    const int64_t nidx = t / tpi, p0 = (t - nidx * tpi) * 64;
    const T* gp = g + nidx * CO * hw + p0;
    const T* rp = r + nidx * CI * hw + p0;
    const T* dp = HAS_D ? d + nidx * CI * hw + p0 : nullptr;
    T* sp = gs ? gs + nidx * CI * hw + p0 : nullptr;
    if (sp) {
      float4 gb[KO];
#pragma unroll
      for (int kk = 0; kk < KO; ++kk)
        gb[kk] = mde::ld4(gp + (4 * kk + q4) * hw + 4 * l16);
#pragma unroll
      for (int mt = 0; mt < MT; ++mt) {
        f4 acc[4];
#pragma unroll
        for (int j = 0; j < 4; ++j) acc[j] = f4{0.f, 0.f, 0.f, 0.f};
#pragma unroll
        for (int kk = 0; kk < KO; ++kk) {
          acc[0] = mfma4(wa[mt][kk], gb[kk].x, acc[0]);
          acc[1] = mfma4(wa[mt][kk], gb[kk].y, acc[1]);
          acc[2] = mfma4(wa[mt][kk], gb[kk].z, acc[2]);
          acc[3] = mfma4(wa[mt][kk], gb[kk].w, acc[3]);
        }
#pragma unroll
        for (int i = 0; i < 4; ++i)
          mde::st4_nt(sp + (16 * mt + 4 * q4 + i) * hw + 4 * l16,
                      make_float4(acc[0][i], acc[1][i], acc[2][i], acc[3][i]));
        if constexpr (BNS) {
#pragma unroll
          for (int i = 0; i < 4; ++i) {
            const float4 x = mde::ld4(rp + (16 * mt + 4 * q4 + i) * hw + 4 * l16);
            const float xv[4] = {x.x, x.y, x.z, x.w};
#pragma unroll
            for (int j = 0; j < 4; ++j) {
              const float e = xv[j] * esc[mt][i] + esh[mt][i] > 0.f ? acc[j][i] : 0.f;
              es1[mt][i] += e;
              es2[mt][i] += e * (xv[j] - emu[mt][i]);
            }
          }
        }
      }
    }
    __builtin_amdgcn_sched_barrier(0);
    constexpr int OG = OT <= 2 ? OT : 1;
#pragma unroll
    for (int og = 0; og < OT; og += OG) {
      float ga[OG][16];
#pragma unroll
      for (int oo = 0; oo < OG; ++oo) {
        const int ot = og + oo;
        const int o = 16 * ot + l16;
        if (o < CO) {
          const T* src = gp + o * hw + 4 * q4;
#pragma unroll
          for (int v = 0; v < 4; ++v) {
            const float4 x = mde::ld4(src + 16 * v);
            ga[oo][4 * v] = x.x; ga[oo][4 * v + 1] = x.y;
            ga[oo][4 * v + 2] = x.z; ga[oo][4 * v + 3] = x.w;
            gbp[ot] += (x.x + x.y) + (x.z + x.w);
          }
        } else {
#pragma unroll
          for (int k = 0; k < 16; ++k) ga[oo][k] = 0.f;
        }
      }
#pragma unroll
      for (int mt = 0; mt < MT; ++mt) {
        const T* ra = rp + (16 * mt + l16) * hw + 4 * q4;
        float sb[16];
#pragma unroll
        for (int v = 0; v < 4; ++v) {
          float4 x = mde::ld4(ra + 16 * v);
          if (BNR) {
            x.x = fmaxf(x.x * bsc[mt] + bsh[mt], 0.f);
            x.y = fmaxf(x.y * bsc[mt] + bsh[mt], 0.f);
            x.z = fmaxf(x.z * bsc[mt] + bsh[mt], 0.f);
            x.w = fmaxf(x.w * bsc[mt] + bsh[mt], 0.f);
          }
          if (HAS_D) {
            const float4 y = mde::ld4(dp + (16 * mt + l16) * hw + 4 * q4 + 16 * v);
            x.x += y.x; x.y += y.y; x.z += y.z; x.w += y.w;
          }
          sb[4 * v] = x.x; sb[4 * v + 1] = x.y; sb[4 * v + 2] = x.z; sb[4 * v + 3] = x.w;
        }
#pragma unroll
        for (int oo = 0; oo < OG; ++oo)
#pragma unroll
          for (int k = 0; k < 16; ++k) gw[og + oo][mt] = mfma4(ga[oo][k], sb[k], gw[og + oo][mt]);
      }
    }
  }
#pragma unroll
  for (int ot = 0; ot < OT; ++ot) {
#pragma unroll
    for (int mt = 0; mt < MT; ++mt)
#pragma unroll
      for (int i = 0; i < 4; ++i) {
        const int o = 16 * ot + 4 * q4 + i;
        if (o < CO) red[w][o * CI + 16 * mt + l16] = gw[ot][mt][i];
      }
    float b = gbp[ot];
    b += __shfl_xor(b, 16, 64);
    b += __shfl_xor(b, 32, 64);
    if (q4 == 0 && 16 * ot + l16 < CO) red[w][CO * CI + 16 * ot + l16] = b;
  }
  if constexpr (BNS) {
#pragma unroll
    for (int mt = 0; mt < MT; ++mt)
#pragma unroll
      for (int i = 0; i < 4; ++i) {
        float a = es1[mt][i], b = es2[mt][i];
#pragma unroll
        for (int o = 1; o < 16; o <<= 1) {
          a += __shfl_xor(a, o, 64);
          b += __shfl_xor(b, o, 64);
        }
        if (l16 == 0) {
          const int c = 16 * mt + 4 * q4 + i;
          red[w][SOFF + 2 * c] = a;
          red[w][SOFF + 2 * c + 1] = b;
        }
      }
  }
  __syncthreads();
  float* out = slab + (int64_t)blockIdx.x * ROW;
  for (int i = threadIdx.x; i < ROW; i += 256)
    out[i] = (red[0][i] + red[1][i]) + (red[2][i] + red[3][i]);
}

template <typename T>
using PwWord = std::conditional_t<std::is_same_v<T, mde::bf16>, uint2, float4>;

template <int CI, int CO, bool BNS, typename T = mde::bf16>
struct PwRaw {
  static constexpr int MT = CI / 16, OT = (CO + 15) / 16, KO = CO / 4;
  static constexpr int OG = OT <= 2 ? OT : 1;
  PwWord<T> gb[KO];
  PwWord<T> ga[OT][4];
  PwWord<T> sr[MT][4];
  PwWord<T> xr[BNS ? MT : 1][4];
};

__device__ __forceinline__ float4 unpack_bf4(uint2 u) {
  return make_float4(__uint_as_float(u.x << 16), __uint_as_float(u.x & 0xffff0000u),
                     __uint_as_float(u.y << 16), __uint_as_float(u.y & 0xffff0000u));
}
__device__ __forceinline__ float4 unpack_bf4(float4 u) { return u; }

template <int CI, int CO, bool BNS, typename T = mde::bf16>
__global__ void __launch_bounds__(256, CI * CO >= 4096 ? 1 : 2)
    pw_bwd_pf_kernel(const T* __restrict__ g, const T* __restrict__ r,
                     const float* __restrict__ wt, T* __restrict__ gs,
                     float* __restrict__ slab, int64_t n, int64_t hw,
                     const float* __restrict__ isc, const float* __restrict__ ish,
                     const float* __restrict__ imean) {
  using Raw = PwRaw<CI, CO, BNS, T>;
  using W = PwWord<T>;
  constexpr int MT = Raw::MT, OT = Raw::OT, KO = Raw::KO, OG = Raw::OG;
  static_assert(CI % 16 == 0 && CO % 8 == 0, "tile shapes");
  static_assert(!BNS || CI <= 32, "BN sums: cin <= 32");
  constexpr int ROW = CO * CI + CO + (BNS ? 2 * CI : 0);
  __shared__ float red[4][ROW];
  const int lane = threadIdx.x & 63, w = threadIdx.x >> 6, l16 = lane & 15, q4 = lane >> 4;
  float wa[MT][KO];
#pragma unroll
  for (int mt = 0; mt < MT; ++mt)
#pragma unroll
    for (int kk = 0; kk < KO; ++kk) wa[mt][kk] = wt[(4 * kk + q4) * CI + 16 * mt + l16];
  f4 gw[OT][MT];
#pragma unroll
  for (int ot = 0; ot < OT; ++ot)
#pragma unroll
    for (int mt = 0; mt < MT; ++mt) gw[ot][mt] = f4{0.f, 0.f, 0.f, 0.f};
  float bsc[MT], bsh[MT];
#pragma unroll
  for (int mt = 0; mt < MT; ++mt) {
    bsc[mt] = isc[16 * mt + l16];
    bsh[mt] = ish[16 * mt + l16];
  }
  constexpr int SOFF = CO * CI + CO;
  float esc[BNS ? MT : 1][4], esh[BNS ? MT : 1][4], emu[BNS ? MT : 1][4];
  float es1[BNS ? MT : 1][4], es2[BNS ? MT : 1][4];
  if constexpr (BNS) {
#pragma unroll
    for (int mt = 0; mt < MT; ++mt)
#pragma unroll
      for (int i = 0; i < 4; ++i) {
        const int c = 16 * mt + 4 * q4 + i;
        esc[mt][i] = isc[c];
        esh[mt][i] = ish[c];
        emu[mt][i] = imean[c];
        es1[mt][i] = 0.f;
        es2[mt][i] = 0.f;
      }
  }
  const int64_t tpi = hw / 64;
  const int64_t tiles = n * tpi;
  const int64_t stride = (int64_t)gridDim.x * 4;
  auto load = [&](int64_t t, Raw& R) {
    if (t >= tiles) t = tiles - 1;
    const int64_t nidx = t / tpi, p0 = (t - nidx * tpi) * 64;
    const T* gp = g + nidx * CO * hw + p0;
    const T* rp = r + nidx * CI * hw + p0;
#pragma unroll
    for (int kk = 0; kk < KO; ++kk)
      R.gb[kk] = *reinterpret_cast<const W*>(gp + (4 * kk + q4) * hw + 4 * l16);
#pragma unroll
    for (int ot = 0; ot < OT; ++ot) {
      const int o = 16 * ot + l16 < CO ? 16 * ot + l16 : CO - 1;
#pragma unroll
      for (int v = 0; v < 4; ++v)
        R.ga[ot][v] = *reinterpret_cast<const W*>(gp + o * hw + 4 * q4 + 16 * v);
    }
#pragma unroll
    for (int mt = 0; mt < MT; ++mt)
#pragma unroll
      for (int v = 0; v < 4; ++v)
        R.sr[mt][v] = *reinterpret_cast<const W*>(rp + (16 * mt + l16) * hw + 4 * q4 + 16 * v);
    if constexpr (BNS) {
#pragma unroll
      for (int mt = 0; mt < MT; ++mt)
#pragma unroll
        for (int i = 0; i < 4; ++i)
          R.xr[mt][i] = *reinterpret_cast<const W*>(rp + (16 * mt + 4 * q4 + i) * hw + 4 * l16);
    }
  };
  auto compute = [&](int64_t t, const Raw& R) {
    const int64_t nidx = t / tpi, p0 = (t - nidx * tpi) * 64;
    T* sp = gs + nidx * CI * hw + p0;
    float4 gb[KO];
#pragma unroll
    for (int kk = 0; kk < KO; ++kk) gb[kk] = unpack_bf4(R.gb[kk]);
#pragma unroll
    for (int mt = 0; mt < MT; ++mt) {
      f4 acc[4];
#pragma unroll
      for (int j = 0; j < 4; ++j) acc[j] = f4{0.f, 0.f, 0.f, 0.f};
#pragma unroll
      for (int kk = 0; kk < KO; ++kk) {
        acc[0] = mfma4(wa[mt][kk], gb[kk].x, acc[0]);
        acc[1] = mfma4(wa[mt][kk], gb[kk].y, acc[1]);
        acc[2] = mfma4(wa[mt][kk], gb[kk].z, acc[2]);
        acc[3] = mfma4(wa[mt][kk], gb[kk].w, acc[3]);
      }
#pragma unroll
      for (int i = 0; i < 4; ++i) {
        if constexpr (std::is_same_v<T, mde::bf16>) {
          using bf2 = __bf16 __attribute__((ext_vector_type(2)));
          const bf2 lo = {(__bf16)acc[0][i], (__bf16)acc[1][i]};
          const bf2 hi = {(__bf16)acc[2][i], (__bf16)acc[3][i]};
          const mde::nt2u u{__builtin_bit_cast(uint32_t, lo), __builtin_bit_cast(uint32_t, hi)};
          __builtin_nontemporal_store(u, reinterpret_cast<mde::nt2u*>(sp + (16 * mt + 4 * q4 + i) * hw + 4 * l16));
        } else {
          mde::st4_nt(sp + (16 * mt + 4 * q4 + i) * hw + 4 * l16,
                      make_float4(acc[0][i], acc[1][i], acc[2][i], acc[3][i]));
        }
      }
      if constexpr (BNS) {
#pragma unroll
        for (int i = 0; i < 4; ++i) {
          const float4 x = unpack_bf4(R.xr[mt][i]);
          const float xv[4] = {x.x, x.y, x.z, x.w};
#pragma unroll
          for (int j = 0; j < 4; ++j) {
            const float e = xv[j] * esc[mt][i] + esh[mt][i] > 0.f ? acc[j][i] : 0.f;
            es1[mt][i] += e;
            es2[mt][i] += e * (xv[j] - emu[mt][i]);
          }
        }
      }
    }
#pragma unroll
    for (int og = 0; og < OT; og += OG) {
      float ga[OG][16];
#pragma unroll
      for (int oo = 0; oo < OG; ++oo) {
        const int ot = og + oo;
        const bool live = 16 * ot + l16 < CO;
#pragma unroll
        for (int v = 0; v < 4; ++v) {
          const float4 x = unpack_bf4(R.ga[ot][v]);
          ga[oo][4 * v] = live ? x.x : 0.f;
          ga[oo][4 * v + 1] = live ? x.y : 0.f;
          ga[oo][4 * v + 2] = live ? x.z : 0.f;
          ga[oo][4 * v + 3] = live ? x.w : 0.f;
        }
      }
#pragma unroll
      for (int mt = 0; mt < MT; ++mt) {
        float sb[16];
#pragma unroll
        for (int v = 0; v < 4; ++v) {
          const float4 x = unpack_bf4(R.sr[mt][v]);
          sb[4 * v] = fmaxf(x.x * bsc[mt] + bsh[mt], 0.f);
          sb[4 * v + 1] = fmaxf(x.y * bsc[mt] + bsh[mt], 0.f);
          sb[4 * v + 2] = fmaxf(x.z * bsc[mt] + bsh[mt], 0.f);
          sb[4 * v + 3] = fmaxf(x.w * bsc[mt] + bsh[mt], 0.f);
        }
#pragma unroll
        for (int oo = 0; oo < OG; ++oo)
#pragma unroll
          for (int k = 0; k < 16; ++k) gw[og + oo][mt] = mfma4(ga[oo][k], sb[k], gw[og + oo][mt]);
      }
    }
  };
  int64_t t = (int64_t)blockIdx.x * 4 + w;
  if (t < tiles) {
    Raw A, B;
    load(t, A);
    while (true) {
      load(t + stride, B);
      compute(t, A);
      t += stride;
      if (t >= tiles) break;
      load(t + stride, A);
      compute(t, B);
      t += stride;
      if (t >= tiles) break;
    }
  }
#pragma unroll
  for (int ot = 0; ot < OT; ++ot)
#pragma unroll
    for (int mt = 0; mt < MT; ++mt)
#pragma unroll
      for (int i = 0; i < 4; ++i) {
        const int o = 16 * ot + 4 * q4 + i;
        if (o < CO) red[w][o * CI + 16 * mt + l16] = gw[ot][mt][i];
      }
  if constexpr (BNS) {
#pragma unroll
    for (int mt = 0; mt < MT; ++mt)
#pragma unroll
      for (int i = 0; i < 4; ++i) {
        float a = es1[mt][i], b = es2[mt][i];
#pragma unroll
        for (int o = 1; o < 16; o <<= 1) {
          a += __shfl_xor(a, o, 64);
          b += __shfl_xor(b, o, 64);
        }
        if (l16 == 0) {
          const int c = 16 * mt + 4 * q4 + i;
          red[w][SOFF + 2 * c] = a;
          red[w][SOFF + 2 * c + 1] = b;
        }
      }
  }
  __syncthreads();
  float* out = slab + (int64_t)blockIdx.x * ROW;
  for (int i = threadIdx.x; i < ROW; i += 256)
    out[i] = (i >= CO * CI && i < SOFF) ? 0.f : (red[0][i] + red[1][i]) + (red[2][i] + red[3][i]);
}

template <int CI, int CO, bool HAS_D, bool BNR = false, bool STATS = false, typename T = float>
__global__ void __launch_bounds__(256)
    skip_fwd_mfma_kernel(const T* __restrict__ r, const T* __restrict__ d,
                         const float* __restrict__ wt, const float* __restrict__ b,
                         T* __restrict__ out, int64_t n, int64_t hw,
                         const float* __restrict__ isc = nullptr,
                         const float* __restrict__ ish = nullptr,
                         float* __restrict__ stats = nullptr, int out_cs = CO) {
  constexpr int OT = (CO + 15) / 16, KC = CI / 4;
  static_assert(CI % 16 == 0 && CO % 8 == 0, "tile shapes");
  constexpr bool HB = HAS_D;
// ... 558 lines not shown
template <int A, int B, typename T>
constexpr bool pw_pf_shape() {
  return A <= 16 && (std::is_same_v<T, mde::bf16> || B <= 16);
}

inline bool pw_pf_on() {
  static const bool on = [] {
    const char* e = std::getenv("MDE_PW_PF");
    return !(e && e[0] == '0');
  }();
  return on;
}

template <typename T>
int pointwise_bwd(const void* gy, const void* x, const float* in_scale, const float* in_shift,
                  const float* in_mean, const float* wt, void* gx, float* gw, float* in_sums,
                  int64_t n, int64_t cin, int64_t cout, int64_t h, int64_t w, void* workspace,
                  hipStream_t s) {
  const int64_t hw = h * w;
  if (!gy || !x || !wt || !gw || !workspace || (!in_scale != !in_shift))
    return MDE_ERR_INVALID_ARG;
  if (!pw_ok(n, cin, cout, hw)) return MDE_ERR_UNSUPPORTED;
  const bool sums = in_sums != nullptr;
  if (sums && (!in_scale || !in_mean || !gx)) return MDE_ERR_INVALID_ARG;
  if (sums && cin > 32) return MDE_ERR_UNSUPPORTED;
  const int nb = bwd_blocks(n, hw);
  float* slab = (float*)workspace;
  const double bytes = (double)sizeof(T) * n * hw * (double)(cout + cin + (gx ? cin : 0));
  const T* gi = (const T*)gy;
  const T* xi = (const T*)x;
  T* go = (T*)gx;
  const bool pf = go != nullptr && pw_pf_on();
  const bool bfp = std::is_same_v<T, mde::bf16> && go != nullptr && pw_bf_on();
  if (bfp) {
    const int rc = mde::pwbf_bwd((const mde::bf16*)gy, (const mde::bf16*)x, in_scale, in_shift,
                                 sums ? in_mean : nullptr, wt, (mde::bf16*)gx, slab, n, cin, cout,
                                 hw, nb, s);
    if (rc != MDE_OK) return rc;
  } else {
#define MDE_PW_BWD(A, B)                                                                     \
  if (cin == A && cout == B && pw_pf_shape<A, B, T>() && pf && in_scale) {                   \
    if constexpr (pw_pf_shape<A, B, T>()) {                                                  \
      if (sums) {                                                                            \
        MDE_LAUNCH(mde::K_PW_BWD, bytes, s, (pw_bwd_pf_kernel<A, B, true, T>), dim3(nb),     \
                   dim3(256), 0, gi, xi, wt, go, slab, n, hw, in_scale, in_shift, in_mean);  \
      } else {                                                                               \
        MDE_LAUNCH(mde::K_PW_BWD, bytes, s, (pw_bwd_pf_kernel<A, B, false, T>), dim3(nb),    \
                   dim3(256), 0, gi, xi, wt, go, slab, n, hw, in_scale, in_shift, nullptr);  \
      }                                                                                      \
    }                                                                                        \
  } else if (cin == A && cout == B) {                                                        \
    if (sums) {                                                                              \
      if constexpr (A <= 32)                                                                 \
        MDE_LAUNCH(mde::K_PW_BWD, bytes, s,                                                  \
                   (skip_bwd_mfma_kernel<A, B, false, true, true, T>), dim3(nb), dim3(256),  \
                   0, gi, xi, nullptr, wt, go, slab, n, hw, in_scale, in_shift, in_mean);    \
    } else if (in_scale) {                                                                   \
      MDE_LAUNCH(mde::K_PW_BWD, bytes, s, (skip_bwd_mfma_kernel<A, B, false, true, false, T>), \
                 dim3(nb), dim3(256), 0, gi, xi, nullptr, wt, go, slab, n, hw, in_scale,     \
                 in_shift, nullptr);                                                         \
    } else {                                                                                 \
      MDE_LAUNCH(mde::K_PW_BWD, bytes, s,                                                    \
                 (skip_bwd_mfma_kernel<A, B, false, false, false, T>), dim3(nb), dim3(256),  \
                 0, gi, xi, nullptr, wt, go, slab, n, hw, nullptr, nullptr, nullptr);        \
    }                                                                                        \
  }
  MDE_PW_SHAPES(MDE_PW_BWD)
#undef MDE_PW_BWD
  }
  const int npairs = (int)(cin * cout), nextra = sums ? 2 * (int)cin : 0;
  const int stride = npairs + (int)cout + nextra;
  if (sums) {
    MDE_LAUNCH(mde::K_PW_BWD, 4.0 * (double)nb * stride, s, skip_slab_reduce_kernel<1>,
               dim3((unsigned)stride), dim3(256), 0, slab, nb, npairs, (int)cout, gw,
               (float*)nullptr, nextra, in_sums);
  } else {
    MDE_LAUNCH(mde::K_PW_BWD, 4.0 * (double)nb * stride, s, skip_slab_reduce_kernel<1>,
               dim3((unsigned)npairs), dim3(256), 0, slab, nb, npairs, (int)cout, gw,
               (float*)nullptr, 0, (float*)nullptr);
  }
  return MDE_OK;
}

}

extern "C" {

int mde_pointwise_bwd(const void* gy, const void* x, const float* in_scale,
                      const float* in_shift, const float* wt, void* gx, float* gw, int64_t n,
                      int64_t cin, int64_t cout, int64_t h, int64_t w, void* workspace,
                      int dtype, void* stream) {
  if (dtype != MDE_F32 && dtype != MDE_BF16) return MDE_ERR_UNSUPPORTED;
  return dtype == MDE_BF16
             ? pointwise_bwd<mde::bf16>(gy, x, in_scale, in_shift, nullptr, wt, gx, gw, nullptr, n,
                                        cin, cout, h, w, workspace, (hipStream_t)stream)
             : pointwise_bwd<float>(gy, x, in_scale, in_shift, nullptr, wt, gx, gw, nullptr, n,
                                    cin, cout, h, w, workspace, (hipStream_t)stream);
}

int mde_pointwise_bwd_bn(const void* gy, const void* x, const float* in_scale,
                         const float* in_shift, const float* in_mean, const float* wt, void* gx,
                         float* gw, float* in_sums, int64_t n, int64_t cin, int64_t cout,
                         int64_t h, int64_t w, void* workspace, int dtype, void* stream) {
  if (dtype != MDE_F32 && dtype != MDE_BF16) return MDE_ERR_UNSUPPORTED;
  if (!in_scale || !in_shift || !in_mean || !gx || !in_sums) return MDE_ERR_INVALID_ARG;
  return dtype == MDE_BF16
             ? pointwise_bwd<mde::bf16>(gy, x, in_scale, in_shift, in_mean, wt, gx, gw, in_sums,
                                        n, cin, cout, h, w, workspace, (hipStream_t)stream)
             : pointwise_bwd<float>(gy, x, in_scale, in_shift, in_mean, wt, gx, gw, in_sums, n,
                                    cin, cout, h, w, workspace, (hipStream_t)stream);
}

}
```

### monocular_depth_estimation_amd/nn.py

```python
from __future__ import annotations

import contextlib
import os

import torch
from torch import nn

from . import _abi
from .functional import GradSlot, _amp_bwd, _amp_fwd, _gpu, _ws

_ACTS = {"none": 0, "relu": 1, "hardswish": 2}


_bn_fwd = torch.amp.custom_fwd(device_type="cuda")


class _BatchNormAct(torch.autograd.Function):
    @staticmethod
    @_bn_fwd
    def forward(ctx, x, weight, bias, prebias, residual, running_mean, running_var, nbt,
                training, momentum, eps, act, stats=None, res_slot=None):
        dt = torch.bfloat16 if x.dtype == torch.bfloat16 else torch.float32
        x = x.to(dt).contiguous()
        residual = residual.to(dt).contiguous() if residual is not None else None
# ... 25 lines not shown
        ctx.training, ctx.act, ctx.has_prebias = bool(training), act, prebias is not None
        ctx.res_slot = res_slot
        return y

    @staticmethod
    @_amp_bwd
    def backward(ctx, gy):
        x, weight, bias, residual, mean, invstd = ctx.saved_tensors
        gy = gy.to(x.dtype).contiguous()
        n, c, h, w = x.shape
        gx = torch.empty_like(x)
        gw = torch.empty_like(weight) if ctx.needs_input_grad[1] else None
        gb = torch.empty_like(bias) if ctx.needs_input_grad[2] else None
        gpb = torch.empty_like(weight) if (ctx.has_prebias and ctx.needs_input_grad[3]) else None
        want_r = residual is not None and ctx.needs_input_grad[4]
        gr = torch.empty_like(x) if (want_r and ctx.act) else None
        ws = _ws(_abi.query("mde_batchnorm_workspace", n, c, h, w), x)
        _abi.call("mde_batchnorm_bwd", _abi.ptr(gy), _abi.ptr(x), _abi.ptr(residual),
                  _abi.ptr(weight), _abi.ptr(bias), _abi.ptr(mean), _abi.ptr(invstd),
                  int(ctx.training), _abi.ptr(gx), _abi.ptr(gr), _abi.ptr(gw), _abi.ptr(gb),
                  _abi.ptr(gpb), n, c, h, w, ctx.act, _abi.ptr(ws), _abi.dtype_code(gy),
                  _abi.stream_of(gy))
        if want_r and not ctx.act:
            gr = gy
        if want_r and ctx.res_slot is not None:
            ctx.res_slot.put(gr)
            gr = None
        return gx, gw, gb, gpb, gr, None, None, None, None, None, None, None, None, None


def batch_norm_act(x, bn: nn.BatchNorm2d, act: str = "none", residual=None, prebias=None,
                   stats=None, res_slot=None):
    _gpu(x, residual, prebias)
    if bn.weight is None or bn.bias is None:
        raise NotImplementedError("affine=False BatchNorm has no HIP kernel")
    training = bn.training or not bn.track_running_stats
    if training and bn.momentum is None:
        raise NotImplementedError("cumulative-average BatchNorm (momentum=None) has no HIP kernel")
    track = bn.training and bn.track_running_stats
    return _BatchNormAct.apply(
        x, bn.weight, bn.bias, prebias, residual,
        bn.running_mean if (track or not training) else None,
        bn.running_var if (track or not training) else None,
        bn.num_batches_tracked if track else None,
        training, bn.momentum if bn.momentum is not None else 0.0, bn.eps, _ACTS[act],
        stats if training else None, res_slot if residual is not None else None)


class _Pointwise(torch.autograd.Function):
    @staticmethod
    @_amp_fwd
    def forward(ctx, x, weight):
        x = x.contiguous()
        n, cin, h, w = x.shape
        cout = weight.shape[0]
        w2 = weight.reshape(cout, cin).contiguous()
        y = torch.empty((n, cout, h, w), dtype=x.dtype, device=x.device)
        _abi.call("mde_pointwise_fwd", _abi.ptr(x), None, None, _abi.ptr(w2), _abi.ptr(y), n, cin,
                  cout, h, w,
                  _abi.dtype_code(x), _abi.stream_of(x))
        ctx.save_for_backward(x, w2)
        ctx.wshape = weight.shape
        return y

    @staticmethod
    @_amp_bwd
    def backward(ctx, gy):
        x, w2 = ctx.saved_tensors
        gy = gy.contiguous()
        n, cin, h, w = x.shape
        cout = w2.shape[0]
        gx = torch.empty_like(x) if ctx.needs_input_grad[0] else None
        gw = torch.empty_like(w2)
        ws = _ws(_abi.query("mde_pointwise_workspace", n, cin, cout, h, w), x)
        _abi.call("mde_pointwise_bwd", _abi.ptr(gy), _abi.ptr(x), None, None, _abi.ptr(w2), _abi.ptr(gx),
                  _abi.ptr(gw), n, cin, cout, h, w, _abi.ptr(ws), _abi.dtype_code(gy),
                  _abi.stream_of(gy))
        return gx, gw.view(ctx.wshape)


_PW_BN_SUMS_MAX_CIN = 32


class _BNReluPointwise(torch.autograd.Function):

    @staticmethod
    @_bn_fwd
    def forward(ctx, y1, gamma, beta, prebias, running_mean, running_var, nbt, training, momentum,
                eps, w2, stats1=None, want_stats2=False):
        y1 = (y1 if y1.dtype == torch.bfloat16 else y1.float()).contiguous()
        n, c, h, w = y1.shape
        cout = w2.shape[0]
        w2m = w2.reshape(cout, c).contiguous()
        f32 = dict(dtype=torch.float32, device=y1.device)
        scale, shift = torch.empty(c, **f32), torch.empty(c, **f32)
        mean, invstd = torch.empty(c, **f32), torch.empty(c, **f32)
        st = _abi.stream_of(y1)
        ws = _ws(_abi.query("mde_batchnorm_workspace", n, c, h, w), y1) if training else None
        if training and stats1 is not None:
            _abi.call("mde_batchnorm_fwd_coef_stats", _abi.ptr(y1), _abi.ptr(gamma),
                      _abi.ptr(beta), _abi.ptr(prebias), _abi.ptr(running_mean),
                      _abi.ptr(running_var), _abi.ptr(nbt), float(momentum), float(eps),
                      _abi.ptr(scale), _abi.ptr(shift), _abi.ptr(mean), _abi.ptr(invstd), n, c, h,
                      w, _abi.ptr(stats1), stats1.shape[1], _abi.ptr(ws), _abi.dtype_code(y1), st)
        else:
            _abi.call("mde_batchnorm_fwd_coef", _abi.ptr(y1), _abi.ptr(gamma), _abi.ptr(beta),
                      _abi.ptr(prebias), _abi.ptr(running_mean), _abi.ptr(running_var),
                      _abi.ptr(nbt), float(momentum), float(eps), int(training), _abi.ptr(scale),
                      _abi.ptr(shift), _abi.ptr(mean), _abi.ptr(invstd), n, c, h, w, _abi.ptr(ws),
                      _abi.dtype_code(y1), st)
        y2 = torch.empty((n, cout, h, w), dtype=y1.dtype, device=y1.device)
        if want_stats2:
            nb = _abi.query("mde_pointwise_stats_blocks", n, c, cout, h, w)
            stats2 = torch.empty((cout, nb, 4), **f32)
            _abi.call("mde_pointwise_fwd_stats", _abi.ptr(y1), _abi.ptr(scale), _abi.ptr(shift),
                      _abi.ptr(w2m), _abi.ptr(y2), _abi.ptr(stats2), n, c, cout, h, w,
                      _abi.dtype_code(y1), st)
        else:
            stats2 = torch.empty((cout, 0, 4), **f32)
            _abi.call("mde_pointwise_fwd", _abi.ptr(y1), _abi.ptr(scale), _abi.ptr(shift),
                      _abi.ptr(w2m), _abi.ptr(y2), n, c, cout, h, w, _abi.dtype_code(y1), st)
        ctx.save_for_backward(y1, gamma, beta, mean, invstd, scale, shift, w2m)
        ctx.training, ctx.has_prebias, ctx.w2shape = bool(training), prebias is not None, w2.shape
        ctx.set_materialize_grads(False)
        ctx.mark_non_differentiable(stats2)
        return y2, stats2

    @staticmethod
    @_amp_bwd
    def backward(ctx, gy2, _gstats2):
        if gy2 is None:
            return (None, None, None, None, None, None, None, None, None, None, None, None, None)
        y1, gamma, beta, mean, invstd, scale, shift, w2m = ctx.saved_tensors
        gy2 = gy2.to(y1.dtype).contiguous()
        n, c, h, w = y1.shape
        cout = w2m.shape[0]
        st = _abi.stream_of(gy2)
        gz = torch.empty_like(y1)
        gw2 = torch.empty_like(w2m)
        ws = _ws(_abi.query("mde_pointwise_workspace", n, c, cout, h, w), y1)
        gy1 = torch.empty_like(y1) if ctx.needs_input_grad[0] else None
        gg = torch.empty_like(gamma)
        gb = torch.empty_like(beta)
        gpb = torch.empty_like(gamma) if (ctx.has_prebias and ctx.needs_input_grad[3]) else None
        gy1_out = gy1 if gy1 is not None else torch.empty_like(y1)
        if c <= _PW_BN_SUMS_MAX_CIN:
            sums = torch.empty((c, 2), dtype=torch.float32, device=y1.device)
            _abi.call("mde_pointwise_bwd_bn", _abi.ptr(gy2), _abi.ptr(y1), _abi.ptr(scale),
                      _abi.ptr(shift), _abi.ptr(mean), _abi.ptr(w2m), _abi.ptr(gz),
                      _abi.ptr(gw2), _abi.ptr(sums), n, c, cout, h, w, _abi.ptr(ws),
                      _abi.dtype_code(gy2), st)
            _abi.call("mde_batchnorm_bwd_apply", _abi.ptr(gz), _abi.ptr(y1), None,
                      _abi.ptr(gamma), _abi.ptr(beta), _abi.ptr(mean), _abi.ptr(invstd),
                      int(ctx.training), _abi.ptr(sums), _abi.ptr(gy1_out), None, _abi.ptr(gg),
                      _abi.ptr(gb), _abi.ptr(gpb), n, c, h, w, _ACTS["relu"],
                      _abi.dtype_code(gy2), st)
        else:
            _abi.call("mde_pointwise_bwd", _abi.ptr(gy2), _abi.ptr(y1), _abi.ptr(scale),
                      _abi.ptr(shift), _abi.ptr(w2m), _abi.ptr(gz), _abi.ptr(gw2), n, c, cout, h,
                      w, _abi.ptr(ws), _abi.dtype_code(gy2), st)
            ws2 = _ws(_abi.query("mde_batchnorm_workspace", n, c, h, w), y1)
            _abi.call("mde_batchnorm_bwd", _abi.ptr(gz), _abi.ptr(y1), None, _abi.ptr(gamma),
                      _abi.ptr(beta), _abi.ptr(mean), _abi.ptr(invstd), int(ctx.training),
                      _abi.ptr(gy1_out), None, _abi.ptr(gg), _abi.ptr(gb), _abi.ptr(gpb), n, c,
                      h, w, _ACTS["relu"], _abi.ptr(ws2), _abi.dtype_code(gy2), st)
        return (gy1, gg, gb, gpb, None, None, None, None, None, None, gw2.view(ctx.w2shape), None,
                None)


def bn_relu_pointwise(y1, bn: nn.BatchNorm2d, prebias, conv: nn.Conv2d, stats1=None,
                      want_stats2=False):
    _gpu(y1, prebias)
    if bn.weight is None or bn.bias is None:
        raise NotImplementedError("affine=False BatchNorm has no HIP kernel")
    training = bn.training or not bn.track_running_stats
    if training and bn.momentum is None:
        raise NotImplementedError("cumulative-average BatchNorm (momentum=None) has no HIP kernel")
    track = bn.training and bn.track_running_stats
    y2, stats2 = _BNReluPointwise.apply(
        y1, bn.weight, bn.bias, prebias,
        bn.running_mean if (track or not training) else None,
        bn.running_var if (track or not training) else None,
        bn.num_batches_tracked if track else None,
        training, bn.momentum if bn.momentum is not None else 0.0, bn.eps, conv.weight,
        stats1 if training else None, bool(want_stats2))
    return y2, (stats2 if stats2.shape[1] > 0 else None)


class _SeBnCat(torch.autograd.Function):

    @staticmethod
    @_bn_fwd
    def forward(ctx, ya, yb, ga, ba, pba, gb, bb, pbb, w1, w2, meta_a, meta_b, sta, stb):
        dt = torch.bfloat16 if torch.bfloat16 in (ya.dtype, yb.dtype) else torch.float32
        ya, yb = ya.to(dt).contiguous(), yb.to(dt).contiguous()
        w1, w2 = w1.contiguous(), w2.contiguous()
        n, ca, h, w = ya.shape
        cb = yb.shape[1]
        c, cr = ca + cb, w1.shape[0]
        f32 = dict(dtype=torch.float32, device=ya.device)
        scale, shift = torch.empty(c, **f32), torch.empty(c, **f32)
        mean, invstd = torch.empty(c, **f32), torch.empty(c, **f32)
        st = _abi.stream_of(ya)
        for y, g, b, pb, meta, stt, lo, hi in ((ya, ga, ba, pba, meta_a, sta, 0, ca),
                                                (yb, gb, bb, pbb, meta_b, stb, ca, c)):
            rm, rv, nbt, momentum, eps = meta
            cc = hi - lo
            ws = _ws(_abi.query("mde_batchnorm_workspace", n, cc, h, w), y)
            views = [t[lo:hi] for t in (scale, shift, mean, invstd)]
            if stt is not None:
                _abi.call("mde_batchnorm_fwd_coef_stats", _abi.ptr(y), _abi.ptr(g), _abi.ptr(b),
                          _abi.ptr(pb), _abi.ptr(rm), _abi.ptr(rv), _abi.ptr(nbt), float(momentum),
                          float(eps), *[_abi.ptr(v) for v in views], n, cc, h, w, _abi.ptr(stt),
                          stt.shape[1], _abi.ptr(ws), _abi.dtype_code(y), st)
            else:
                _abi.call("mde_batchnorm_fwd_coef", _abi.ptr(y), _abi.ptr(g), _abi.ptr(b),
                          _abi.ptr(pb), _abi.ptr(rm), _abi.ptr(rv), _abi.ptr(nbt), float(momentum),
                          float(eps), 1, *[_abi.ptr(v) for v in views], n, cc, h, w, _abi.ptr(ws),
                          _abi.dtype_code(y), st)
        out = torch.empty((n, c, h, w), dtype=dt, device=ya.device)
        s, hidden, semean = torch.empty((n, c), **f32), torch.empty((n, cr), **f32), torch.empty((n, c), **f32)
        ws = _ws(_abi.query("mde_se_bn_workspace", n, c, cr, h, w), ya)
        _abi.call("mde_se_bn_fwd", _abi.ptr(ya), ca, _abi.ptr(yb), cb, _abi.ptr(scale),
                  _abi.ptr(shift), _abi.ptr(w1), _abi.ptr(w2), cr, _abi.ptr(out), _abi.ptr(s),
                  _abi.ptr(hidden), _abi.ptr(semean), n, h, w, _abi.ptr(ws), _abi.dtype_code(ya), st)
        ctx.save_for_backward(ya, yb, w1, w2, scale, shift, mean, invstd, s, hidden, semean)
        ctx.has_pb = (pba is not None, pbb is not None)
        return out

    @staticmethod
    @_amp_bwd
    def backward(ctx, gout):
        ya, yb, w1, w2, scale, shift, mean, invstd, s, hidden, semean = ctx.saved_tensors
        gout = gout.to(ya.dtype).contiguous()
        n, ca, h, w = ya.shape
        c, cr = ca + yb.shape[1], w1.shape[0]
        gya, gyb = torch.empty_like(ya), torch.empty_like(yb)
        gg, gbt = torch.empty_like(scale), torch.empty_like(scale)
        gw1, gw2 = torch.empty_like(w1), torch.empty_like(w2)
        ws = _ws(_abi.query("mde_se_bn_workspace", n, c, cr, h, w), ya)
        _abi.call("mde_se_bn_bwd", _abi.ptr(gout), _abi.ptr(ya), ca, _abi.ptr(yb), c - ca,
                  _abi.ptr(scale), _abi.ptr(shift), _abi.ptr(mean), _abi.ptr(invstd), 1,
                  _abi.ptr(w1), _abi.ptr(w2), cr, _abi.ptr(s), _abi.ptr(hidden), _abi.ptr(semean),
                  _abi.ptr(gya), _abi.ptr(gyb), _abi.ptr(gg), _abi.ptr(gbt), _abi.ptr(gw1),
                  _abi.ptr(gw2), n, h, w, _abi.ptr(ws), _abi.dtype_code(gout), _abi.stream_of(gout))
        zpa = torch.zeros(ca, dtype=torch.float32, device=ya.device) if ctx.has_pb[0] else None
        zpb = torch.zeros(c - ca, dtype=torch.float32, device=ya.device) if ctx.has_pb[1] else None
        return (gya, gyb, gg[:ca], gbt[:ca], zpa, gg[ca:], gbt[ca:], zpb, gw1, gw2, None, None,
                None, None)


def se_bn_cat(ya, yb, bn_a: nn.BatchNorm2d, bn_b: nn.BatchNorm2d, pb_a, pb_b, w1, w2,
              stats_a=None, stats_b=None):
    _gpu(ya, yb, pb_a, pb_b, w1, w2)
    for bn in (bn_a, bn_b):
        if bn.weight is None or bn.bias is None or bn.momentum is None or not bn.training:
            raise NotImplementedError("se_bn_cat needs affine, momentum, training-mode BatchNorms")

    def meta(bn):
        track = bn.track_running_stats
        return (bn.running_mean if track else None, bn.running_var if track else None,
                bn.num_batches_tracked if track else None, bn.momentum, bn.eps)

    return _SeBnCat.apply(ya, yb, bn_a.weight, bn_a.bias, pb_a, bn_b.weight, bn_b.bias, pb_b,
                          w1, w2, meta(bn_a), meta(bn_b), stats_a, stats_b)


def pointwise_ok(conv: nn.Conv2d, x) -> bool:
    if (conv.kernel_size != (1, 1) or conv.stride != (1, 1) or conv.padding != (0, 0)
            or conv.dilation != (1, 1) or conv.groups != 1 or x.dim() != 4
            or conv.weight.dtype != torch.float32):
        return False
    return bool(_abi.query("mde_pointwise_supported", conv.in_channels, conv.out_channels,
                           x.shape[2], x.shape[3]))


CONV3X3_HIP = {
    (3, 16): (True, True, True),
    (3, 32): (True, True, True),
    (3, 64): (True, True, True),
    (16, 16): (True, True, True),
    (32, 32): (False, False, True),
}
WIDE_WGRAD_ALL = os.environ.get("MDE_WIDE_WGRAD", "1") != "0"
WIDE_PAD = os.environ.get("MDE_WIDE_PAD", "1") != "0"
WINO_MIN_BLOCKS = int(os.environ.get("MDE_WINO_MIN_BLOCKS", "256"))
if WIDE_WGRAD_ALL:
    CONV3X3_HIP.update({(64, 64): (False, False, True), (128, 64): (False, False, True),
                        (128, 128): (False, False, True), (256, 256): (False, False, True)})


class _Conv3x3(torch.autograd.Function):
    @staticmethod
    @_amp_fwd
    def forward(ctx, x, weight, passes, want_stats=False, gx_slot=None):
        wkey = weight
        x = x.contiguous()
        weight = weight.contiguous()
        n, cin, h, w = x.shape
        cout = weight.shape[0]
        stats = torch.empty((cout, 0, 4), dtype=torch.float32, device=x.device)
        ctx.gx_slot = gx_slot
        u_flip = None
        if passes[0] == WINO:
            y = torch.empty((n, cout, h, w), dtype=x.dtype, device=x.device)
            st = _abi.stream_of(x)
            if want_stats:
                nb = _abi.query("mde_wino_stats_blocks", n, cin, cout, h, w)
                stats = torch.empty((cout, nb, 4), dtype=torch.float32, device=x.device)
            flip = passes[1] == WINO
            sc = _ACTIVE_PACK
            ent = sc.wino.get(wkey) if sc is not None else None
            if ent is not None and wkey in sc.wino_packed and (ent[1] is not None or not flip):
                u, u_flip = ent[0], (ent[1] if flip else None)
            else:
                ub = _abi.query("mde_wino_weight_bytes", cin, cout) // 4
                u = torch.empty(ub, dtype=torch.float32, device=x.device)
                if flip:
                    u_flip = torch.empty(ub, dtype=torch.float32, device=x.device)
                    _abi.call("mde_wino_weight2", _abi.ptr(weight), _abi.ptr(u), _abi.ptr(u_flip),
                              cin, cout, st)
                else:
                    _abi.call("mde_wino_weight", _abi.ptr(weight), _abi.ptr(u), cin, cout, 0, st)
                if (sc is not None and ent is None and isinstance(wkey, nn.Parameter)
                        and not torch.cuda.is_current_stream_capturing()):
                    sc.wino[wkey] = (u, u_flip, cin, cout)
            _abi.call("mde_wino_conv_stats", _abi.ptr(x), _abi.ptr(u), _abi.ptr(y),
                      _abi.ptr(stats) if want_stats else None, n, cin, cout, h, w, 0,
                      _abi.dtype_code(x), st)
        elif passes[0] == WIDE:
            y = torch.empty((n, cout, h, w), dtype=x.dtype, device=x.device)
            _abi.call("mde_conv3x3_wide_fwd", _abi.ptr(x), _abi.ptr(weight), _abi.ptr(y), n, cin,
                      cout, h, w, _abi.dtype_code(x), _abi.stream_of(x))
        elif passes[0]:
            y = torch.empty((n, cout, h, w), dtype=x.dtype, device=x.device)
            if want_stats:
                nb = _abi.query("mde_conv3x3_stats_blocks", n, cin, cout, h, w, _abi.MDE_F32)
                stats = torch.empty((cout, nb, 4), dtype=torch.float32, device=x.device)
                _abi.call("mde_conv3x3_fwd_stats", _abi.ptr(x), _abi.ptr(weight), _abi.ptr(y),
                          _abi.ptr(stats), n, cin, cout, h, w, _abi.dtype_code(x),
                          _abi.stream_of(x))
            else:
                _abi.call("mde_conv3x3_fwd", _abi.ptr(x), _abi.ptr(weight), _abi.ptr(y), n, cin,
                          cout, h, w, _abi.dtype_code(x), _abi.stream_of(x))
        else:
            y = torch.nn.functional.conv2d(x, weight, None, 1, 1)
        ctx.save_for_backward(x, weight)
        ctx.passes = passes
# ... 815 lines not shown
                    return _BiasAdd.apply(y, self.bias)
                return y + self.bias.view(1, -1, 1, 1)
        return super().forward(x)


def _bnrelu_pw_at(mods, i, x_shape) -> bool:
    if i + 4 >= len(mods):
        return False
    c0, b0, r0, c1, b1 = mods[i:i + 5]
    return (isinstance(c0, nn.Conv2d) and c0.bias is not None and c0.padding_mode == "zeros"
            and isinstance(b0, BatchNorm2d) and b0.act == "relu"
            and isinstance(r0, nn.Identity)
            and isinstance(c1, nn.Conv2d) and c1.bias is not None and isinstance(b1, BatchNorm2d)
            and c1.kernel_size == (1, 1) and c1.stride == (1, 1) and c1.padding == (0, 0)
            and c1.groups == 1 and c1.in_channels == c0.out_channels)


def run_sequential(seq: nn.Sequential, x):
    mods = list(seq)
    i = 0
    while i < len(mods):
        m = mods[i]
        if x.is_cuda and _bnrelu_pw_at(mods, i, x.shape):
            want = mods[i + 1].training or not mods[i + 1].track_running_stats
            passes = conv3x3_passes(m, x)
            if passes is not None and want:
                y1, st1 = conv3x3_stats(x, m.weight, passes)
            else:
                y1, st1 = conv_nobias(m, x), None
            if pointwise_ok(mods[i + 3], y1):
                b2 = mods[i + 4]
                y2, st2 = bn_relu_pointwise(y1, mods[i + 1], m.bias, mods[i + 3], st1,
                                            b2.training or not b2.track_running_stats)
                x = batch_norm_act(y2, b2, b2.act, None, mods[i + 3].bias, st2)
                i += 5
                continue
            x = batch_norm_act(y1, mods[i + 1], mods[i + 1].act, None, m.bias, st1)
            i += 2
            continue
        if (isinstance(m, nn.Conv2d) and m.bias is not None and i + 1 < len(mods)
                and isinstance(mods[i + 1], BatchNorm2d) and m.padding_mode == "zeros"):
            x = conv_bn(m, mods[i + 1], x)
            i += 2
        elif (isinstance(m, Conv2d) and m.bias is None and i + 1 < len(mods)
              and isinstance(mods[i + 1], BatchNorm2d) and m.padding_mode == "zeros"):
            y, st = conv_nobias_stats(m, x, mods[i + 1])
            x = mods[i + 1](y, stats=st)
            i += 2
        else:
            x = m(x)
            i += 1
    return x


def run_sequential_raw(seq: nn.Sequential, x):
    mods = list(seq)
    if (len(mods) != 6 or not x.is_cuda or x.dtype not in (torch.float32, torch.bfloat16)
            or not _bnrelu_pw_at(mods, 0, x.shape)
            or not isinstance(mods[5], nn.Identity) or mods[4].act != "relu"
            or not mods[1].training or not mods[4].training):
        return None
    m, c1 = mods[0], mods[3]
    k = m.kernel_size
    same = (m.stride == (1, 1) and m.dilation == (1, 1) and k[0] % 2 == 1 and k[1] % 2 == 1
            and m.padding == (k[0] // 2, k[1] // 2))
    passes = conv3x3_passes(m, x)
    if passes is not None:
        y1, st1 = conv3x3_stats(x, m.weight, passes)
    else:
        y1, st1 = conv_nobias(m, x), None
    if same and pointwise_ok(c1, x):
        y2, st2 = bn_relu_pointwise(y1, mods[1], m.bias, c1, st1, True)
        return y2, st2, mods[4], c1.bias
    x1 = batch_norm_act(y1, mods[1], "relu", None, m.bias, st1)
    y2 = torch.nn.functional.conv2d(x1, c1.weight, None, c1.stride, c1.padding, c1.dilation,
                                    c1.groups)
    return y2, None, mods[4], c1.bias


class _SkipReduceBN(torch.autograd.Function):

    @staticmethod
    @_bn_fwd
    def forward(ctx, r, d, weight, bias, gamma, beta, prebias, meta, stats, d_slot=None):
        dt = torch.bfloat16 if r.dtype == torch.bfloat16 else torch.float32
        r, d = r.to(dt).contiguous(), d.to(dt).contiguous()
        n, cin, h, w = r.shape
        cout = weight.shape[0]
        wm = weight.reshape(cout, cin).contiguous()
        f32 = dict(dtype=torch.float32, device=r.device)
        scale, shift = torch.empty(cin, **f32), torch.empty(cin, **f32)
        mean, invstd = torch.empty(cin, **f32), torch.empty(cin, **f32)
        rm, rv, nbt, momentum, eps = meta
        st = _abi.stream_of(r)
        ws = _ws(_abi.query("mde_batchnorm_workspace", n, cin, h, w), r)
        if stats is not None:
            _abi.call("mde_batchnorm_fwd_coef_stats", _abi.ptr(r), _abi.ptr(gamma), _abi.ptr(beta),
                      _abi.ptr(prebias), _abi.ptr(rm), _abi.ptr(rv), _abi.ptr(nbt), float(momentum),
                      float(eps), _abi.ptr(scale), _abi.ptr(shift), _abi.ptr(mean), _abi.ptr(invstd),
                      n, cin, h, w, _abi.ptr(stats), stats.shape[1], _abi.ptr(ws),
                      _abi.dtype_code(r), st)
        else:
            _abi.call("mde_batchnorm_fwd_coef", _abi.ptr(r), _abi.ptr(gamma), _abi.ptr(beta),
                      _abi.ptr(prebias), _abi.ptr(rm), _abi.ptr(rv), _abi.ptr(nbt), float(momentum),
                      float(eps), 1, _abi.ptr(scale), _abi.ptr(shift), _abi.ptr(mean),
                      _abi.ptr(invstd), n, cin, h, w, _abi.ptr(ws), _abi.dtype_code(r), st)
        out = torch.empty((n, cout, h, w), dtype=dt, device=r.device)
        _abi.call("mde_skip_reduce_bn_fwd", _abi.ptr(r), _abi.ptr(d), _abi.ptr(scale),
                  _abi.ptr(shift), _abi.ptr(wm), _abi.ptr(bias), _abi.ptr(out), n, cin, cout, h, w,
                  _abi.dtype_code(r), st)
        ctx.save_for_backward(r, d, wm, gamma, beta, scale, shift, mean, invstd)
        ctx.wshape, ctx.has_pb, ctx.d_slot = weight.shape, prebias is not None, d_slot
        return out

    @staticmethod
    @_amp_bwd
    def backward(ctx, gout):
        r, d, wm, gamma, beta, scale, shift, mean, invstd = ctx.saved_tensors
        gout = gout.to(r.dtype).contiguous()
        n, cin, h, w = r.shape
        cout = wm.shape[0]
        st = _abi.stream_of(gout)
        gs = torch.empty_like(r)
        gw, gb = torch.empty_like(wm), torch.empty(cout, dtype=torch.float32, device=r.device)
        use_sums = bool(_abi.query("mde_skip_reduce_bn_supported", cin, cout, h, w, 1))
        sums = torch.empty((cin, 2), dtype=torch.float32, device=r.device) if use_sums else None
        ws = _ws(_abi.query("mde_skip_reduce_bn_workspace", n, cin, cout, h, w), r)
        _abi.call("mde_skip_reduce_bn_bwd", _abi.ptr(gout), _abi.ptr(r), _abi.ptr(d),
                  _abi.ptr(scale), _abi.ptr(shift), _abi.ptr(mean), _abi.ptr(wm), _abi.ptr(gs),
                  _abi.ptr(gw), _abi.ptr(gb), _abi.ptr(sums), n, cin, cout, h, w, _abi.ptr(ws),
                  _abi.dtype_code(gout), st)
        gr = torch.empty_like(r)
        gg, gbeta = torch.empty_like(gamma), torch.empty_like(beta)
        gpb = torch.empty_like(gamma) if (ctx.has_pb and ctx.needs_input_grad[6]) else None
        if sums is not None:
            _abi.call("mde_batchnorm_bwd_apply", _abi.ptr(gs), _abi.ptr(r), None, _abi.ptr(gamma),
                      _abi.ptr(beta), _abi.ptr(mean), _abi.ptr(invstd), 1, _abi.ptr(sums),
                      _abi.ptr(gr), None, _abi.ptr(gg), _abi.ptr(gbeta), _abi.ptr(gpb), n, cin, h,
                      w, _ACTS["relu"], _abi.dtype_code(gout), st)
        else:
            ws2 = _ws(_abi.query("mde_batchnorm_workspace", n, cin, h, w), r)
            _abi.call("mde_batchnorm_bwd", _abi.ptr(gs), _abi.ptr(r), None, _abi.ptr(gamma),
                      _abi.ptr(beta), _abi.ptr(mean), _abi.ptr(invstd), 1, _abi.ptr(gr), None,
                      _abi.ptr(gg), _abi.ptr(gbeta), _abi.ptr(gpb), n, cin, h, w, _ACTS["relu"],
                      _abi.ptr(ws2), _abi.dtype_code(gout), st)
        if ctx.d_slot is not None and ctx.needs_input_grad[1]:
            ctx.d_slot.put(gs)
            gd = None
        else:
            gd = gs
        return gr, gd, gw.view(ctx.wshape), gb, gg, gbeta, gpb, None, None, None


def skip_reduce_bn_ok(r, cout: int) -> bool:
    return (r.dim() == 4 and r.dtype in (torch.float32, torch.bfloat16) and
            bool(_abi.query("mde_skip_reduce_bn_supported", r.shape[1], cout, r.shape[2],
                            r.shape[3], 0)))


def skip_reduce_bn(r, bn: nn.BatchNorm2d, prebias, d, weight, bias, stats=None):
    _gpu(r, d, prebias, weight, bias)
    if bn.weight is None or bn.bias is None or bn.momentum is None or not bn.training:
        raise NotImplementedError("skip_reduce_bn needs an affine, momentum, training-mode BatchNorm")
    track = bn.track_running_stats
    meta = (bn.running_mean if track else None, bn.running_var if track else None,
            bn.num_batches_tracked if track else None, bn.momentum, bn.eps)
    return _SkipReduceBN.apply(r, d, weight, bias, bn.weight, bn.bias, prebias, meta, stats,
                               getattr(d, "_mde_grad_slot", None))


class BatchNorm2d(nn.BatchNorm2d):

    def __init__(self, num_features, eps=1e-5, momentum=0.1, act="none", **kw):
        super().__init__(num_features, eps=eps, momentum=momentum, **kw)
        if act not in _ACTS:
            raise ValueError(f"act must be one of {sorted(_ACTS)}")
        self.act = act

    def forward(self, x, residual=None, prebias=None, stats=None, act=None, res_slot=None):
        return batch_norm_act(x, self, self.act if act is None else act, residual, prebias, stats,
                              res_slot)

    def extra_repr(self):
        return super().extra_repr() + f", act={self.act}"


class _DWConv(torch.autograd.Function):
    @staticmethod
    @_amp_fwd
    def forward(ctx, x, weight, k, stride, pad):
        x = x.contiguous()
        n, c, h, w = x.shape
        ho, wo = (h + 2 * pad - k) // stride + 1, (w + 2 * pad - k) // stride + 1
        y = torch.empty((n, c, ho, wo), dtype=x.dtype, device=x.device)
        _abi.call("mde_dwconv_fwd", _abi.ptr(x), _abi.ptr(weight), _abi.ptr(y), n, c, h, w, k,
                  stride, pad, _abi.dtype_code(x), _abi.stream_of(x))
        ctx.save_for_backward(x, weight)
        ctx.meta = (k, stride, pad)
        return y

    @staticmethod
    @_amp_bwd
    def backward(ctx, gy):
        x, weight = ctx.saved_tensors
        k, stride, pad = ctx.meta
        gy = gy.contiguous()
        n, c, h, w = x.shape
        gx = torch.empty_like(x) if ctx.needs_input_grad[0] else None
        gw = torch.empty_like(weight) if ctx.needs_input_grad[1] else None
        ws = _ws(_abi.query("mde_dwconv_workspace", n, c, h, w, k, stride, pad), x) \
            if gw is not None else None
        if gx is not None or gw is not None:
            _abi.call("mde_dwconv_bwd", _abi.ptr(gy), _abi.ptr(x), _abi.ptr(weight), _abi.ptr(gx),
                      _abi.ptr(gw), n, c, h, w, k, stride, pad, _abi.ptr(ws),
                      _abi.dtype_code(gy), _abi.stream_of(gy))
        return gx, gw, None, None, None


def depthwise_conv2d(x, conv: nn.Conv2d):
    _gpu(x)
    k = conv.kernel_size[0]
    s = conv.stride[0]
    p = conv.padding[0]
    if (conv.kernel_size != (k, k) or k not in (3, 5) or conv.stride != (s, s) or s not in (1, 2)
            or conv.padding != (p, p) or conv.dilation != (1, 1) or conv.padding_mode != "zeros"
            or not (conv.groups == conv.in_channels == conv.out_channels)):
        raise NotImplementedError(f"no HIP depthwise kernel for {conv}")
    y = _DWConv.apply(x, conv.weight, k, s, p)
    if conv.bias is not None:
        y = y + conv.bias.view(1, -1, 1, 1)
    return y


def depthwise_conv_bn_act(x, conv: nn.Conv2d, bn: "BatchNorm2d", act: str = "none"):
    return batch_norm_act(depthwise_conv2d(x, conv), bn, act)


class _SEGate(torch.autograd.Function):
    @staticmethod
    @_amp_fwd
    def forward(ctx, x, w1, b1, w2, b2):
        x = x.contiguous()
        n, c, h, w = x.shape
        cr = w1.shape[0]
        ctx.wshapes = (w1.shape, w2.shape)
        w1 = w1.reshape(cr, c).contiguous()
        w2 = w2.reshape(c, cr).contiguous()
        out = torch.empty_like(x)
        s = torch.empty((n, c), dtype=torch.float32, device=x.device)
        hidden = torch.empty((n, cr), dtype=torch.float32, device=x.device)
        mean = torch.empty((n, c), dtype=torch.float32, device=x.device)
# ... 33 lines not shown
```

Before: 1002 images/s.

## Defer BN/SE backward apply into the downstream pointwise-conv backward kernel

The BN backward in skip_reduce_bn and the SE+BN backward in se_bn_cat now only compute per-channel coefficient tables. The elementwise gradient apply that used to write a full gradient tensor is handed through a slot to the preceding pointwise-conv backward, which applies it on load inside its MFMA kernel via shared-memory tiles. This removes a full read/write pass over large activation gradients per fused block. The cost is extra shared memory and register pressure in the pointwise backward kernel, and more complex slot-based coupling between autograd functions that only covers the fp32 path.

```diff
diff --git a/include/mde_abi.h b/include/mde_abi.h
--- a/include/mde_abi.h
+++ b/include/mde_abi.h
@@ -77,6 +77,13 @@
                   int64_t cr, const float* s, const float* hidden, const float* mean, void* gya,
                   void* gyb, float* ggamma, float* gbeta, float* gw1, float* gw2, int64_t n,
                   int64_t h, int64_t w, void* workspace, int dtype, void* stream);
+int mde_se_bn_bwd_coef(const void* gout, const void* ya, int64_t ca, const void* yb, int64_t cb,
+                       const float* scale, const float* shift, const float* bn_mean,
+                       const float* bn_invstd, int training, const float* w1, const float* w2,
+                       int64_t cr, const float* s, const float* hidden, const float* mean,
+                       float* dm, float* tab, float* ggamma, float* gbeta, float* gw1,
+                       float* gw2, int64_t n, int64_t h, int64_t w, void* workspace, int dtype,
+                       void* stream);
 
 int mde_skip_reduce_fwd(const void* r, const void* d, const float* wt,
                         const float* b, void* out, int64_t n, int64_t cin,
@@ -170,6 +177,10 @@
                             void* gresidual, float* ggamma, float* gbeta, float* gprebias,
                             int64_t n, int64_t c, int64_t h, int64_t w, int act, int dtype,
                             void* stream);
+int mde_batchnorm_bwd_coef(const float* gamma, const float* beta, const float* mean,
+                           const float* invstd, int training, const float* sums, float* tab,
+                           float* ggamma, float* gbeta, float* gprebias, int64_t n, int64_t c,
+                           int64_t h, int64_t w, void* stream);
 
 size_t mde_window_attn_workspace(int64_t b, int64_t h, int64_t w, int64_t c,
                                  int64_t heads, int64_t window);
@@ -224,6 +235,14 @@
                          void* gx, float* gweight, float* in_sums, int64_t n, int64_t cin,
                          int64_t cout, int64_t h, int64_t w, void* workspace, int dtype,
                          void* stream);
+int mde_pointwise_deferred_supported(int64_t cin, int64_t cout, int64_t h, int64_t w);
+int mde_pointwise_bwd_bn_deferred(const void* g_raw, int64_t g_channels, int64_t g_choff,
+                                  const void* y_out, const float* tab, const float* se_s,
+                                  const float* se_dm, const void* x, const float* in_scale,
+                                  const float* in_shift, const float* in_mean,
+                                  const float* weight, void* gx, float* gweight, float* in_sums,
+                                  int64_t n, int64_t cin, int64_t cout, int64_t h, int64_t w,
+                                  void* workspace, int dtype, void* stream);
 
 int mde_conv3x3_supported(int64_t cin, int64_t cout, int pass, int dtype);
 int mde_conv3x3_fwd(const void* x, const float* weight, void* y, int64_t n, int64_t cin,
diff --git a/monocular_depth_estimation_amd/_abi.py b/monocular_depth_estimation_amd/_abi.py
--- a/monocular_depth_estimation_amd/_abi.py
+++ b/monocular_depth_estimation_amd/_abi.py
@@ -97,6 +97,15 @@
                                             _int, _vp]),
     "mde_pointwise_bwd_bn": (_int, [_vp, _vp, _vp, _vp, _vp, _vp, _vp, _vp, _vp, _i64, _i64, _i64,
                                     _i64, _i64, _vp, _int, _vp]),
+    "mde_pointwise_deferred_supported": (_int, [_i64, _i64, _i64, _i64]),
+    "mde_pointwise_bwd_bn_deferred": (_int, [_vp, _i64, _i64, _vp, _vp, _vp, _vp, _vp, _vp, _vp, _vp,
+                                             _vp, _vp, _vp, _vp, _i64, _i64, _i64, _i64, _i64, _vp,
+                                             _int, _vp]),
+    "mde_batchnorm_bwd_coef": (_int, [_vp, _vp, _vp, _vp, _int, _vp, _vp, _vp, _vp, _vp, _i64, _i64,
+                                      _i64, _i64, _vp]),
+    "mde_se_bn_bwd_coef": (_int, [_vp, _vp, _i64, _vp, _i64, _vp, _vp, _vp, _vp, _int, _vp, _vp, _i64,
+                                  _vp, _vp, _vp, _vp, _vp, _vp, _vp, _vp, _vp, _i64, _i64, _i64, _vp,
+                                  _int, _vp]),
     "mde_batchnorm_fwd_coef": (_int, [_vp, _vp, _vp, _vp, _vp, _vp, _vp, _f32, _f32, _int, _vp, _vp,
                                       _vp, _vp, _i64, _i64, _i64, _i64, _vp, _int, _vp]),
     "mde_conv3x3_supported": (_int, [_i64, _i64, _int, _int]),
diff --git a/monocular_depth_estimation_amd/csrc/bn.hip b/monocular_depth_estimation_amd/csrc/bn.hip
--- a/monocular_depth_estimation_amd/csrc/bn.hip
+++ b/monocular_depth_estimation_amd/csrc/bn.hip
@@ -465,6 +465,18 @@
   return r;
 }
 
+__global__ void __launch_bounds__(256)
+    bn_bwd_coef_kernel(int64_t c, BwdArgs P, float* __restrict__ tab) {
+  const int64_t ch = blockIdx.x * (int64_t)blockDim.x + threadIdx.x;
+  if (ch >= c) return;
+  const BwdCh k = bwd_channel(P, ch, (double)P.part[2 * ch], (double)P.part[2 * ch + 1], true);
+  tab[ch] = k.sc;
+  tab[c + ch] = k.sh;
+  tab[2 * c + ch] = k.A;
+  tab[3 * c + ch] = k.B;
+  tab[4 * c + ch] = k.D;
+}
+
 template <typename T>
 __global__ void __launch_bounds__(256)
     bn_bwd_apply_plane_kernel(const T* __restrict__ gy, const T* __restrict__ x,
@@ -1143,4 +1155,16 @@
              : bwd_apply<float>(gy, x, residual, gx, gresidual, n, c, hw, act, P, s);
 }
 
-}
+int mde_batchnorm_bwd_coef(const float* gamma, const float* beta, const float* mean,
+                           const float* invstd, int training, const float* sums, float* tab,
+                           float* ggamma, float* gbeta, float* gprebias, int64_t n, int64_t c,
+                           int64_t h, int64_t w, void* stream) {
+  if (!gamma || !beta || !mean || !invstd || !sums || !tab || !args_ok(n, c, h, w))
+    return MDE_ERR_INVALID_ARG;
+  BwdArgs P{gamma, beta, mean, invstd, sums, 1, n * h * w, training, ggamma, gbeta, gprebias};
+  MDE_LAUNCH(mde::K_BN_BWD_FINAL, 4.0 * 14.0 * (double)c, (hipStream_t)stream, bn_bwd_coef_kernel,
+             dim3((unsigned)mde::cdiv(c, 256)), dim3(256), 0, c, P, tab);
+  return MDE_OK;
+}
+
+}
diff --git a/monocular_depth_estimation_amd/csrc/se.hip b/monocular_depth_estimation_amd/csrc/se.hip
--- a/monocular_depth_estimation_amd/csrc/se.hip
+++ b/monocular_depth_estimation_amd/csrc/se.hip
@@ -354,7 +354,10 @@
                             float* __restrict__ coef, int cr, const float* __restrict__ w1,
                             const float* __restrict__ dz, const float* __restrict__ dh,
                             const float* __restrict__ hidden, const float* __restrict__ mean,
-                            float* __restrict__ gw1, float* __restrict__ gw2) {
+                            float* __restrict__ gw1, float* __restrict__ gw2,
+                            const float* __restrict__ bn_shift = nullptr,
+                            const float* __restrict__ bn_mean = nullptr,
+                            float* __restrict__ tab = nullptr) {
   __shared__ double red[2][4];
   __shared__ float dms[kMaxSeN];
   if ((int64_t)blockIdx.x >= c) {
@@ -409,6 +412,13 @@
   if (gbeta) gbeta[ch] = (float)s1;
   coef[2 * ch] = training ? (float)(-sc * s1 / cnt) : 0.f;
   coef[2 * ch + 1] = training ? (float)(-sc * is * is * s2 / cnt) : 0.f;
+  if (tab) {
+    tab[ch] = scale[ch];
+    tab[c + ch] = bn_shift[ch];
+    tab[2 * c + ch] = bn_mean[ch];
+    tab[3 * c + ch] = coef[2 * ch + 1];
+    tab[4 * c + ch] = coef[2 * ch];
+  }
 }
 
 template <typename T = float>
@@ -654,9 +664,11 @@
                        const float* bn_invstd, int training, const float* w1, const float* w2,
                        int64_t cr, const float* s, const float* hidden, const float* mean,
                        void* gya, void* gyb, float* ggamma, float* gbeta, float* gw1, float* gw2,
-                       int64_t n, int64_t hw, void* workspace, hipStream_t st) {
+                       int64_t n, int64_t hw, void* workspace, hipStream_t st,
+                       float* dm_out = nullptr, float* tab = nullptr) {
   const int64_t c = ca + cb;
   SeWs ws = se_carve(workspace, n, c, cr, hw);
+  if (dm_out) ws.dm = dm_out;
   const int chunks = (int)se_chunks(hw);
   const double big = (double)sizeof(T) * n * c * (double)hw;
   MDE_LAUNCH(mde::K_SE_BWD_DOT, 2.0 * big, st, sebn_bwd_reduce_kernel<T>,
@@ -669,7 +681,8 @@
              st, sebn_bwd_combine_kernel,
              dim3((unsigned)(c + mde::cdiv(2 * c * cr, 256))), dim3(256), 0, ws.part4, chunks, n, c,
              hw, s, ws.dm, scale, bn_invstd, training, ggamma, gbeta, ws.coef, (int)cr, w1, ws.dz,
-             ws.dh, hidden, mean, gw1, gw2);
+             ws.dh, hidden, mean, gw1, gw2, shift, bn_mean, tab);
+  if (tab) return MDE_OK;
   MDE_LAUNCH(mde::K_SE_BWD_APPLY, 3.0 * big, st, sebn_bwd_apply_kernel<T>,
              dim3(stream_grid(n * c * hw / 4)), dim3(256), 0, (const T*)gout, (const T*)ya, ca,
              (const T*)yb, cb, hw, n * c, s, ws.dm, 1.f / (float)hw, scale, shift, bn_mean,
@@ -720,4 +733,22 @@
                                   gw1, gw2, n, hw, workspace, st);
 }
 
-}
+int mde_se_bn_bwd_coef(const void* gout, const void* ya, int64_t ca, const void* yb, int64_t cb,
+                       const float* scale, const float* shift, const float* bn_mean,
+                       const float* bn_invstd, int training, const float* w1, const float* w2,
+                       int64_t cr, const float* s, const float* hidden, const float* mean,
+                       float* dm, float* tab, float* ggamma, float* gbeta, float* gw1, float* gw2,
+                       int64_t n, int64_t h, int64_t w, void* workspace, int dtype, void* stream) {
+  if (dtype != MDE_F32) return MDE_ERR_UNSUPPORTED;
+  const int64_t c = ca + cb, hw = h * w;
+  if (!gout || !ya || ca <= 0 || cb < 0 || (cb > 0 && !yb) || !scale || !shift || !bn_mean ||
+      !bn_invstd || !w1 || !w2 || cr <= 0 || !s || !hidden || !mean || !dm || !tab || !gw1 ||
+      !gw2 || n <= 0 || hw <= 0 || !workspace || c > 4096 || cr > 4096 || n > 65535 ||
+      n * c > 65535)
+    return MDE_ERR_INVALID_ARG;
+  return se_bn_bwd_t<float>(gout, ya, ca, yb, cb, scale, shift, bn_mean, bn_invstd, training, w1,
+                            w2, cr, s, hidden, mean, nullptr, nullptr, ggamma, gbeta, gw1, gw2, n,
+                            hw, workspace, (hipStream_t)stream, dm, tab);
+}
+
+}
diff --git a/monocular_depth_estimation_amd/csrc/skip.hip b/monocular_depth_estimation_amd/csrc/skip.hip
--- a/monocular_depth_estimation_amd/csrc/skip.hip
+++ b/monocular_depth_estimation_amd/csrc/skip.hip
@@ -275,20 +275,78 @@
   return __builtin_amdgcn_mfma_f32_16x16x4f32(a, b, c, 0, 0, 0);
 }
 
-template <int CI, int CO, bool HAS_D, bool BNR = false, bool BNS = false, typename T = float>
+struct PwDefer {
+  const float* y;
+  const float* tab;
+  const float* s;
+  const float* dm;
+  float inv_hw;
+  int tstride;
+  int64_t gpitch;
+};
+
+constexpr int kPwGPitch = 68;
+
+struct PwDeferCo {
+  float sc, sh, c2, c3, c4, P, Q;
+};
+
+template <int DEF>
+__device__ __forceinline__ float pw_defer1(float g, float y, const PwDeferCo& k) {
+#pragma clang fp contract(off)
+  if constexpr (DEF == 1) {
+    const float e = fmaf(y, k.sc, k.sh) > 0.f ? g : 0.f;
+    return fmaf(k.c3, y, k.c2 * e) + k.c4;
+  } else {
+    const float z = fmaf(y, k.sc, k.sh);
+    return (z > 0.f ? fmaf(k.P, g, k.Q) : 0.f) + fmaf(k.c3, y - k.c2, k.c4);
+  }
+}
+
+template <int DEF>
+__device__ __forceinline__ float4 pw_defer4(float4 g, float4 y, const PwDeferCo& k) {
+  return make_float4(pw_defer1<DEF>(g.x, y.x, k), pw_defer1<DEF>(g.y, y.y, k),
+                     pw_defer1<DEF>(g.z, y.z, k), pw_defer1<DEF>(g.w, y.w, k));
+}
+
+template <int DEF, int CO>
+__device__ __forceinline__ PwDeferCo pw_defer_co(const float (*dt)[CO], int o, float sv, float dv,
+                                                 float inv_hw) {
+  PwDeferCo k{dt[0][o], dt[1][o], dt[2][o], dt[3][o], dt[4][o], 0.f, 0.f};
+  if constexpr (DEF == 2) {
+    k.P = k.sc * sv;
+    k.Q = k.sc * dv * inv_hw;
+  }
+  return k;
+}
+
+template <int CI, int CO, bool HAS_D, bool BNR = false, bool BNS = false, typename T = float,
+          int DEF = 0>
 __global__ void __launch_bounds__(256, CI * CO >= 4096 ? 1 : 2)
     skip_bwd_mfma_kernel(const T* __restrict__ g, const T* __restrict__ r,
                          const T* __restrict__ d, const float* __restrict__ wt,
                          T* __restrict__ gs, float* __restrict__ slab, int64_t n,
                          int64_t hw, const float* __restrict__ isc = nullptr,
                          const float* __restrict__ ish = nullptr,
-                         const float* __restrict__ imean = nullptr) {
+                         const float* __restrict__ imean = nullptr, PwDefer df = {}) {
+  static_assert(DEF == 0 || std::is_same_v<T, float>, "deferred gradient: fp32 storage");
   constexpr int MT = CI / 16, OT = (CO + 15) / 16, KO = CO / 4;
   static_assert(CI % 16 == 0 && CO % 8 == 0, "tile shapes");
   static_assert(!BNS || (BNR && CI <= 32), "BN sums: fused BN-ReLU operand, cin <= 32");
   constexpr int ROW = CO * CI + CO + (BNS ? 2 * CI : 0);
   __shared__ float red[4][ROW];
   const int lane = threadIdx.x & 63, w = threadIdx.x >> 6, l16 = lane & 15, q4 = lane >> 4;
+  const float(*dt)[CO] = nullptr;
+  float* gt = nullptr;
+  if constexpr (DEF != 0) {
+    __shared__ float dtab[5][CO];
+    __shared__ __attribute__((aligned(16))) float gtile[4][CO * kPwGPitch];
+    for (int i = threadIdx.x; i < 5 * CO; i += 256)
+      dtab[i / CO][i % CO] = df.tab[(i / CO) * df.tstride + i % CO];
+    __syncthreads();
+    dt = dtab;
+    gt = gtile[w];
+  }
   float wa[MT][KO];
 #pragma unroll
   for (int mt = 0; mt < MT; ++mt)
@@ -326,15 +384,37 @@
   const int64_t tiles = n * tpi;
   for (int64_t t = (int64_t)blockIdx.x * 4 + w; t < tiles; t += (int64_t)gridDim.x * 4) {
     const int64_t nidx = t / tpi, p0 = (t - nidx * tpi) * 64;
-    const T* gp = g + nidx * CO * hw + p0;
+    const T* gp = g + (DEF != 0 ? nidx * df.gpitch : nidx * CO * hw) + p0;
     const T* rp = r + nidx * CI * hw + p0;
     const T* dp = HAS_D ? d + nidx * CI * hw + p0 : nullptr;
     T* sp = gs ? gs + nidx * CI * hw + p0 : nullptr;
+    const float* yp = DEF != 0 ? df.y + nidx * CO * hw + p0 : nullptr;
     if (sp) {
       float4 gb[KO];
 #pragma unroll
       for (int kk = 0; kk < KO; ++kk)
         gb[kk] = mde::ld4(gp + (4 * kk + q4) * hw + 4 * l16);
+      if constexpr (DEF != 0) {
+        float4 yb[KO];
+        float sv[KO] = {}, dv[KO] = {};
+#pragma unroll
+        for (int kk = 0; kk < KO; ++kk) {
+          yb[kk] = mde::ld4(yp + (4 * kk + q4) * hw + 4 * l16);
+          if constexpr (DEF == 2) {
+            sv[kk] = df.s[nidx * df.tstride + 4 * kk + q4];
+            dv[kk] = df.dm[nidx * df.tstride + 4 * kk + q4];
+          }
+        }
+#pragma unroll
+        for (int kk = 0; kk < KO; ++kk)
+          gb[kk] = pw_defer4<DEF>(
+              gb[kk], yb[kk], pw_defer_co<DEF, CO>(dt, 4 * kk + q4, sv[kk], dv[kk], df.inv_hw));
+        __builtin_amdgcn_wave_barrier();
+#pragma unroll
+        for (int kk = 0; kk < KO; ++kk)
+          *reinterpret_cast<float4*>(gt + (4 * kk + q4) * kPwGPitch + 4 * l16) = gb[kk];
+        __builtin_amdgcn_wave_barrier();
+      }
 #pragma unroll
       for (int mt = 0; mt < MT; ++mt) {
         f4 acc[4];
@@ -379,7 +459,11 @@
           const T* src = gp + o * hw + 4 * q4;
 #pragma unroll
           for (int v = 0; v < 4; ++v) {
-            const float4 x = mde::ld4(src + 16 * v);
+            float4 x;
+            if constexpr (DEF != 0)
+              x = *reinterpret_cast<const float4*>(gt + o * kPwGPitch + 4 * q4 + 16 * v);
+            else
+              x = mde::ld4(src + 16 * v);
             ga[oo][4 * v] = x.x; ga[oo][4 * v + 1] = x.y;
             ga[oo][4 * v + 2] = x.z; ga[oo][4 * v + 3] = x.w;
             gbp[ot] += (x.x + x.y) + (x.z + x.w);
@@ -456,14 +540,16 @@
 template <typename T>
 using PwWord = std::conditional_t<std::is_same_v<T, mde::bf16>, uint2, float4>;
 
-template <int CI, int CO, bool BNS, typename T = mde::bf16>
+template <int CI, int CO, bool BNS, typename T = mde::bf16, int DEF = 0>
 struct PwRaw {
   static constexpr int MT = CI / 16, OT = (CO + 15) / 16, KO = CO / 4;
   static constexpr int OG = OT <= 2 ? OT : 1;
   PwWord<T> gb[KO];
-  PwWord<T> ga[OT][4];
+  PwWord<T> ga[DEF ? 1 : OT][4];
   PwWord<T> sr[MT][4];
   PwWord<T> xr[BNS ? MT : 1][4];
+  PwWord<T> yb[DEF ? KO : 1];
+  float sb[DEF == 2 ? KO : 1], db[DEF == 2 ? KO : 1];
 };
 
 __device__ __forceinline__ float4 unpack_bf4(uint2 u) {
@@ -472,21 +558,33 @@
 }
 __device__ __forceinline__ float4 unpack_bf4(float4 u) { return u; }
 
-template <int CI, int CO, bool BNS, typename T = mde::bf16>
+template <int CI, int CO, bool BNS, typename T = mde::bf16, int DEF = 0>
 __global__ void __launch_bounds__(256, CI * CO >= 4096 ? 1 : 2)
     pw_bwd_pf_kernel(const T* __restrict__ g, const T* __restrict__ r,
                      const float* __restrict__ wt, T* __restrict__ gs,
                      float* __restrict__ slab, int64_t n, int64_t hw,
                      const float* __restrict__ isc, const float* __restrict__ ish,
-                     const float* __restrict__ imean) {
-  using Raw = PwRaw<CI, CO, BNS, T>;
+                     const float* __restrict__ imean, PwDefer df = {}) {
+  using Raw = PwRaw<CI, CO, BNS, T, DEF>;
   using W = PwWord<T>;
+  static_assert(DEF == 0 || std::is_same_v<T, float>, "deferred gradient: fp32 storage");
   constexpr int MT = Raw::MT, OT = Raw::OT, KO = Raw::KO, OG = Raw::OG;
   static_assert(CI % 16 == 0 && CO % 8 == 0, "tile shapes");
   static_assert(!BNS || CI <= 32, "BN sums: cin <= 32");
   constexpr int ROW = CO * CI + CO + (BNS ? 2 * CI : 0);
   __shared__ float red[4][ROW];
   const int lane = threadIdx.x & 63, w = threadIdx.x >> 6, l16 = lane & 15, q4 = lane >> 4;
+  const float(*dt)[CO] = nullptr;
+  float* gt = nullptr;
+  if constexpr (DEF != 0) {
+    __shared__ float dtab[5][CO];
+    __shared__ __attribute__((aligned(16))) float gtile[4][CO * kPwGPitch];
+    for (int i = threadIdx.x; i < 5 * CO; i += 256)
+      dtab[i / CO][i % CO] = df.tab[(i / CO) * df.tstride + i % CO];
+    __syncthreads();
+    dt = dtab;
+    gt = gtile[w];
+  }
   float wa[MT][KO];
 #pragma unroll
   for (int mt = 0; mt < MT; ++mt)
@@ -525,17 +623,30 @@
   auto load = [&](int64_t t, Raw& R) {
     if (t >= tiles) t = tiles - 1;
     const int64_t nidx = t / tpi, p0 = (t - nidx * tpi) * 64;
-    const T* gp = g + nidx * CO * hw + p0;
+    const T* gp = g + (DEF != 0 ? nidx * df.gpitch : nidx * CO * hw) + p0;
     const T* rp = r + nidx * CI * hw + p0;
 #pragma unroll
     for (int kk = 0; kk < KO; ++kk)
       R.gb[kk] = *reinterpret_cast<const W*>(gp + (4 * kk + q4) * hw + 4 * l16);
-#pragma unroll
-    for (int ot = 0; ot < OT; ++ot) {
-      const int o = 16 * ot + l16 < CO ? 16 * ot + l16 : CO - 1;
-#pragma unroll
-      for (int v = 0; v < 4; ++v)
-        R.ga[ot][v] = *reinterpret_cast<const W*>(gp + o * hw + 4 * q4 + 16 * v);
+    if constexpr (DEF == 0) {
+#pragma unroll
+      for (int ot = 0; ot < OT; ++ot) {
+        const int o = 16 * ot + l16 < CO ? 16 * ot + l16 : CO - 1;
+#pragma unroll
+        for (int v = 0; v < 4; ++v)
+          R.ga[ot][v] = *reinterpret_cast<const W*>(gp + o * hw + 4 * q4 + 16 * v);
+      }
+    }
+    if constexpr (DEF != 0) {
+      const float* yp = df.y + nidx * CO * hw + p0;
+#pragma unroll
+      for (int kk = 0; kk < KO; ++kk) {
+        R.yb[kk] = *reinterpret_cast<const W*>(yp + (4 * kk + q4) * hw + 4 * l16);
+        if constexpr (DEF == 2) {
+          R.sb[kk] = df.s[nidx * df.tstride + 4 * kk + q4];
+          R.db[kk] = df.dm[nidx * df.tstride + 4 * kk + q4];
+        }
+      }
     }
 #pragma unroll
     for (int mt = 0; mt < MT; ++mt)
@@ -555,7 +666,20 @@
     T* sp = gs + nidx * CI * hw + p0;
     float4 gb[KO];
 #pragma unroll
-    for (int kk = 0; kk < KO; ++kk) gb[kk] = unpack_bf4(R.gb[kk]);
+    for (int kk = 0; kk < KO; ++kk) {
+      gb[kk] = unpack_bf4(R.gb[kk]);
+      if constexpr (DEF != 0)
+        gb[kk] = pw_defer4<DEF>(gb[kk], unpack_bf4(R.yb[kk]),
+                                pw_defer_co<DEF, CO>(dt, 4 * kk + q4, DEF == 2 ? R.sb[kk] : 0.f,
+                                                     DEF == 2 ? R.db[kk] : 0.f, df.inv_hw));
+    }
+    if constexpr (DEF != 0) {
+      __builtin_amdgcn_wave_barrier();
+#pragma unroll
+      for (int kk = 0; kk < KO; ++kk)
+        *reinterpret_cast<float4*>(gt + (4 * kk + q4) * kPwGPitch + 4 * l16) = gb[kk];
+      __builtin_amdgcn_wave_barrier();
+    }
 #pragma unroll
     for (int mt = 0; mt < MT; ++mt) {
       f4 acc[4];
@@ -604,7 +728,12 @@
         const bool live = 16 * ot + l16 < CO;
 #pragma unroll
         for (int v = 0; v < 4; ++v) {
-          const float4 x = unpack_bf4(R.ga[ot][v]);
+          float4 x;
+          if constexpr (DEF != 0)
+            x = *reinterpret_cast<const float4*>(
+                gt + (live ? 16 * ot + l16 : CO - 1) * kPwGPitch + 4 * q4 + 16 * v);
+          else
+            x = unpack_bf4(R.ga[ot][v]);
           ga[oo][4 * v] = live ? x.x : 0.f;
           ga[oo][4 * v + 1] = live ? x.y : 0.f;
           ga[oo][4 * v + 2] = live ? x.z : 0.f;
@@ -1329,9 +1458,95 @@
   return MDE_OK;
 }
 
+#define MDE_PW_DEFER_SHAPES(X) X(16, 8) X(16, 16) X(16, 32) X(32, 16) X(32, 32)
+
+bool pw_defer_ok(int64_t n, int64_t cin, int64_t cout, int64_t hw) {
+  if (n <= 0 || hw <= 0 || hw % 64 != 0) return false;
+#define MDE_PW_MATCH(A, B) if (cin == A && cout == B) return true;
+  MDE_PW_DEFER_SHAPES(MDE_PW_MATCH)
+#undef MDE_PW_MATCH
+  return false;
+}
+
+template <int DEF>
+int pointwise_bwd_deferred(const float* g, const float* x, const float* in_scale,
+                           const float* in_shift, const float* in_mean, const float* wt,
+                           float* gx, float* gw, float* in_sums, int64_t n, int64_t cin,
+                           int64_t cout, int64_t hw, void* workspace, const PwDefer& df,
+                           hipStream_t s) {
+  const int nb = bwd_blocks(n, hw);
+  float* slab = (float*)workspace;
+  const double bytes = 4.0 * n * hw * (double)(2 * cout + 2 * cin);
+  const bool pf = pw_pf_on();
+#define MDE_PW_DEF(A, B)                                                                     \
+  if (cin == A && cout == B) {                                                                \
+    if constexpr (pw_pf_shape<A, B, float>()) {                                               \
+      if (pf) {                                                                               \
+        MDE_LAUNCH(mde::K_PW_BWD, bytes, s, (pw_bwd_pf_kernel<A, B, true, float, DEF>),       \
+                   dim3(nb), dim3(256), 0, g, x, wt, gx, slab, n, hw, in_scale, in_shift,     \
+                   in_mean, df);                                                              \
+      } else {                                                                                \
+        MDE_LAUNCH(mde::K_PW_BWD, bytes, s,                                                   \
+                   (skip_bwd_mfma_kernel<A, B, false, true, true, float, DEF>), dim3(nb),     \
+                   dim3(256), 0, g, x, nullptr, wt, gx, slab, n, hw, in_scale, in_shift,      \
+                   in_mean, df);                                                              \
+      }                                                                                       \
+    } else {                                                                                  \
+      MDE_LAUNCH(mde::K_PW_BWD, bytes, s,                                                     \
+                 (skip_bwd_mfma_kernel<A, B, false, true, true, float, DEF>), dim3(nb),       \
+                 dim3(256), 0, g, x, nullptr, wt, gx, slab, n, hw, in_scale, in_shift,        \
+                 in_mean, df);                                                                \
+    }                                                                                         \
+  }
+  MDE_PW_DEFER_SHAPES(MDE_PW_DEF)
+#undef MDE_PW_DEF
+  const int npairs = (int)(cin * cout), nextra = 2 * (int)cin;
+  const int stride = npairs + (int)cout + nextra;
+  MDE_LAUNCH(mde::K_PW_BWD, 4.0 * (double)nb * stride, s, skip_slab_reduce_kernel<1>,
+             dim3((unsigned)stride), dim3(256), 0, slab, nb, npairs, (int)cout, gw,
+             (float*)nullptr, nextra, in_sums);
+  return MDE_OK;
+}
+
 }
 
 extern "C" {
+
+int mde_pointwise_deferred_supported(int64_t cin, int64_t cout, int64_t h, int64_t w) {
+  return pw_defer_ok(1, cin, cout, h * w) ? 1 : 0;
+}
+
+int mde_pointwise_bwd_bn_deferred(const void* g_raw, int64_t g_channels, int64_t g_choff,
+                                  const void* y_out, const float* tab, const float* se_s,
+                                  const float* se_dm, const void* x, const float* in_scale,
+                                  const float* in_shift, const float* in_mean, const float* wt,
+                                  void* gx, float* gw, float* in_sums, int64_t n, int64_t cin,
+                                  int64_t cout, int64_t h, int64_t w, void* workspace, int dtype,
+                                  void* stream) {
+  if (dtype != MDE_F32) return MDE_ERR_UNSUPPORTED;
+  const int64_t hw = h * w;
+  if (!g_raw || !y_out || !tab || !x || !in_scale || !in_shift || !in_mean || !wt || !gx || !gw ||
+      !in_sums || !workspace || (!se_s != !se_dm) || g_choff < 0 || g_choff + cout > g_channels ||
+      g_channels > INT32_MAX)
+    return MDE_ERR_INVALID_ARG;
+  if (!pw_defer_ok(n, cin, cout, hw)) return MDE_ERR_UNSUPPORTED;
+  PwDefer df;
+  df.y = (const float*)y_out;
+  df.tab = tab + g_choff;
+  df.s = se_s ? se_s + g_choff : nullptr;
+  df.dm = se_dm ? se_dm + g_choff : nullptr;
+  df.inv_hw = 1.f / (float)hw;
+  df.tstride = (int)g_channels;
+  df.gpitch = g_channels * hw;
+  const float* g = (const float*)g_raw + g_choff * hw;
+  hipStream_t s = (hipStream_t)stream;
+  return se_s ? pointwise_bwd_deferred<2>(g, (const float*)x, in_scale, in_shift, in_mean, wt,
+                                          (float*)gx, gw, in_sums, n, cin, cout, hw, workspace,
+                                          df, s)
+              : pointwise_bwd_deferred<1>(g, (const float*)x, in_scale, in_shift, in_mean, wt,
+                                          (float*)gx, gw, in_sums, n, cin, cout, hw, workspace,
+                                          df, s);
+}
 
 int mde_pointwise_bwd(const void* gy, const void* x, const float* in_scale,
                       const float* in_shift, const float* wt, void* gx, float* gw, int64_t n,
diff --git a/monocular_depth_estimation_amd/nn.py b/monocular_depth_estimation_amd/nn.py
--- a/monocular_depth_estimation_amd/nn.py
+++ b/monocular_depth_estimation_amd/nn.py
@@ -131,12 +131,39 @@
 _PW_BN_SUMS_MAX_CIN = 32
 
 
+class PwGradSlot:
+
+    __slots__ = ("payload",)
+
+    def __init__(self):
+        self.payload = None
+
+    def put(self, g_raw, choff, y_out, tab, se_s=None, se_dm=None):
+        self.payload = (g_raw, choff, y_out, tab, se_s, se_dm)
+
+    def take(self):
+        p, self.payload = self.payload, None
+        return p
+
+
+def _pw_defer_slot(y1, cout, training):
+    if os.environ.get("MDE_PW_DEFER", "1") == "0":
+        return None
+    if not (training and y1.dtype == torch.float32 and y1.requires_grad
+            and torch.is_grad_enabled()):
+        return None
+    n, c, h, w = y1.shape
+    if c > _PW_BN_SUMS_MAX_CIN or not _abi.query("mde_pointwise_deferred_supported", c, cout, h, w):
+        return None
+    return PwGradSlot()
+
+
 class _BNReluPointwise(torch.autograd.Function):
 
     @staticmethod
     @_bn_fwd
     def forward(ctx, y1, gamma, beta, prebias, running_mean, running_var, nbt, training, momentum,
-                eps, w2, stats1=None, want_stats2=False):
+                eps, w2, stats1=None, want_stats2=False, defer_slot=None):
         y1 = (y1 if y1.dtype == torch.bfloat16 else y1.float()).contiguous()
         n, c, h, w = y1.shape
         cout = w2.shape[0]
@@ -171,6 +198,7 @@
                       _abi.ptr(w2m), _abi.ptr(y2), n, c, cout, h, w, _abi.dtype_code(y1), st)
         ctx.save_for_backward(y1, gamma, beta, mean, invstd, scale, shift, w2m)
         ctx.training, ctx.has_prebias, ctx.w2shape = bool(training), prebias is not None, w2.shape
+        ctx.defer_slot = defer_slot
         ctx.set_materialize_grads(False)
         ctx.mark_non_differentiable(stats2)
         return y2, stats2
@@ -179,9 +207,11 @@
     @_amp_bwd
     def backward(ctx, gy2, _gstats2):
         if gy2 is None:
-            return (None, None, None, None, None, None, None, None, None, None, None, None, None)
+            return (None,) * 14
         y1, gamma, beta, mean, invstd, scale, shift, w2m = ctx.saved_tensors
-        gy2 = gy2.to(y1.dtype).contiguous()
+        deferred = ctx.defer_slot.take() if ctx.defer_slot is not None else None
+        if deferred is None:
+            gy2 = gy2.to(y1.dtype).contiguous()
         n, c, h, w = y1.shape
         cout = w2m.shape[0]
         st = _abi.stream_of(gy2)
@@ -195,10 +225,18 @@
         gy1_out = gy1 if gy1 is not None else torch.empty_like(y1)
         if c <= _PW_BN_SUMS_MAX_CIN:
             sums = torch.empty((c, 2), dtype=torch.float32, device=y1.device)
-            _abi.call("mde_pointwise_bwd_bn", _abi.ptr(gy2), _abi.ptr(y1), _abi.ptr(scale),
-                      _abi.ptr(shift), _abi.ptr(mean), _abi.ptr(w2m), _abi.ptr(gz),
-                      _abi.ptr(gw2), _abi.ptr(sums), n, c, cout, h, w, _abi.ptr(ws),
-                      _abi.dtype_code(gy2), st)
+            if deferred is not None:
+                g_raw, choff, y_out, tab, se_s, se_dm = deferred
+                _abi.call("mde_pointwise_bwd_bn_deferred", _abi.ptr(g_raw), g_raw.shape[1], choff,
+                          _abi.ptr(y_out), _abi.ptr(tab), _abi.ptr(se_s), _abi.ptr(se_dm),
+                          _abi.ptr(y1), _abi.ptr(scale), _abi.ptr(shift), _abi.ptr(mean),
+                          _abi.ptr(w2m), _abi.ptr(gz), _abi.ptr(gw2), _abi.ptr(sums), n, c, cout,
+                          h, w, _abi.ptr(ws), _abi.dtype_code(y1), st)
+            else:
+                _abi.call("mde_pointwise_bwd_bn", _abi.ptr(gy2), _abi.ptr(y1), _abi.ptr(scale),
+                          _abi.ptr(shift), _abi.ptr(mean), _abi.ptr(w2m), _abi.ptr(gz),
+                          _abi.ptr(gw2), _abi.ptr(sums), n, c, cout, h, w, _abi.ptr(ws),
+                          _abi.dtype_code(gy2), st)
             _abi.call("mde_batchnorm_bwd_apply", _abi.ptr(gz), _abi.ptr(y1), None,
                       _abi.ptr(gamma), _abi.ptr(beta), _abi.ptr(mean), _abi.ptr(invstd),
                       int(ctx.training), _abi.ptr(sums), _abi.ptr(gy1_out), None, _abi.ptr(gg),
@@ -214,7 +252,7 @@
                       _abi.ptr(gy1_out), None, _abi.ptr(gg), _abi.ptr(gb), _abi.ptr(gpb), n, c,
                       h, w, _ACTS["relu"], _abi.ptr(ws2), _abi.dtype_code(gy2), st)
         return (gy1, gg, gb, gpb, None, None, None, None, None, None, gw2.view(ctx.w2shape), None,
-                None)
+                None, None)
 
 
 def bn_relu_pointwise(y1, bn: nn.BatchNorm2d, prebias, conv: nn.Conv2d, stats1=None,
@@ -226,13 +264,16 @@
     if training and bn.momentum is None:
         raise NotImplementedError("cumulative-average BatchNorm (momentum=None) has no HIP kernel")
     track = bn.training and bn.track_running_stats
+    slot = _pw_defer_slot(y1, conv.weight.shape[0], training)
     y2, stats2 = _BNReluPointwise.apply(
         y1, bn.weight, bn.bias, prebias,
         bn.running_mean if (track or not training) else None,
         bn.running_var if (track or not training) else None,
         bn.num_batches_tracked if track else None,
         training, bn.momentum if bn.momentum is not None else 0.0, bn.eps, conv.weight,
-        stats1 if training else None, bool(want_stats2))
+        stats1 if training else None, bool(want_stats2), slot)
+    if slot is not None:
+        y2._mde_pw_slot = slot
     return y2, (stats2 if stats2.shape[1] > 0 else None)
 
 
@@ -240,7 +281,8 @@
 
     @staticmethod
     @_bn_fwd
-    def forward(ctx, ya, yb, ga, ba, pba, gb, bb, pbb, w1, w2, meta_a, meta_b, sta, stb):
+    def forward(ctx, ya, yb, ga, ba, pba, gb, bb, pbb, w1, w2, meta_a, meta_b, sta, stb,
+                pw_slots=None):
         dt = torch.bfloat16 if torch.bfloat16 in (ya.dtype, yb.dtype) else torch.float32
         ya, yb = ya.to(dt).contiguous(), yb.to(dt).contiguous()
         w1, w2 = w1.contiguous(), w2.contiguous()
@@ -275,6 +317,7 @@
                   _abi.ptr(hidden), _abi.ptr(semean), n, h, w, _abi.ptr(ws), _abi.dtype_code(ya), st)
         ctx.save_for_backward(ya, yb, w1, w2, scale, shift, mean, invstd, s, hidden, semean)
         ctx.has_pb = (pba is not None, pbb is not None)
+        ctx.pw_slots = pw_slots if dt == torch.float32 else None
         return out
 
     @staticmethod
@@ -284,19 +327,33 @@
         gout = gout.to(ya.dtype).contiguous()
         n, ca, h, w = ya.shape
         c, cr = ca + yb.shape[1], w1.shape[0]
-        gya, gyb = torch.empty_like(ya), torch.empty_like(yb)
         gg, gbt = torch.empty_like(scale), torch.empty_like(scale)
         gw1, gw2 = torch.empty_like(w1), torch.empty_like(w2)
         ws = _ws(_abi.query("mde_se_bn_workspace", n, c, cr, h, w), ya)
+        zpa = torch.zeros(ca, dtype=torch.float32, device=ya.device) if ctx.has_pb[0] else None
+        zpb = torch.zeros(c - ca, dtype=torch.float32, device=ya.device) if ctx.has_pb[1] else None
+        if (ctx.pw_slots is not None and ctx.needs_input_grad[0] and ctx.needs_input_grad[1]
+                and gout.dtype == torch.float32):
+            dm = torch.empty((n, c), dtype=torch.float32, device=ya.device)
+            tab = torch.empty((5, c), dtype=torch.float32, device=ya.device)
+            _abi.call("mde_se_bn_bwd_coef", _abi.ptr(gout), _abi.ptr(ya), ca, _abi.ptr(yb), c - ca,
+                      _abi.ptr(scale), _abi.ptr(shift), _abi.ptr(mean), _abi.ptr(invstd), 1,
+                      _abi.ptr(w1), _abi.ptr(w2), cr, _abi.ptr(s), _abi.ptr(hidden),
+                      _abi.ptr(semean), _abi.ptr(dm), _abi.ptr(tab), _abi.ptr(gg), _abi.ptr(gbt),
+                      _abi.ptr(gw1), _abi.ptr(gw2), n, h, w, _abi.ptr(ws), _abi.dtype_code(gout),
+                      _abi.stream_of(gout))
+            ctx.pw_slots[0].put(gout, 0, ya, tab, s, dm)
+            ctx.pw_slots[1].put(gout, ca, yb, tab, s, dm)
+            return (gout[:, :ca], gout[:, ca:], gg[:ca], gbt[:ca], zpa, gg[ca:], gbt[ca:], zpb,
+                    gw1, gw2, None, None, None, None, None)
+        gya, gyb = torch.empty_like(ya), torch.empty_like(yb)
         _abi.call("mde_se_bn_bwd", _abi.ptr(gout), _abi.ptr(ya), ca, _abi.ptr(yb), c - ca,
                   _abi.ptr(scale), _abi.ptr(shift), _abi.ptr(mean), _abi.ptr(invstd), 1,
                   _abi.ptr(w1), _abi.ptr(w2), cr, _abi.ptr(s), _abi.ptr(hidden), _abi.ptr(semean),
                   _abi.ptr(gya), _abi.ptr(gyb), _abi.ptr(gg), _abi.ptr(gbt), _abi.ptr(gw1),
                   _abi.ptr(gw2), n, h, w, _abi.ptr(ws), _abi.dtype_code(gout), _abi.stream_of(gout))
-        zpa = torch.zeros(ca, dtype=torch.float32, device=ya.device) if ctx.has_pb[0] else None
-        zpb = torch.zeros(c - ca, dtype=torch.float32, device=ya.device) if ctx.has_pb[1] else None
         return (gya, gyb, gg[:ca], gbt[:ca], zpa, gg[ca:], gbt[ca:], zpb, gw1, gw2, None, None,
-                None, None)
+                None, None, None)
 
 
 def se_bn_cat(ya, yb, bn_a: nn.BatchNorm2d, bn_b: nn.BatchNorm2d, pb_a, pb_b, w1, w2,
@@ -311,8 +368,10 @@
         return (bn.running_mean if track else None, bn.running_var if track else None,
                 bn.num_batches_tracked if track else None, bn.momentum, bn.eps)
 
+    slots = (getattr(ya, "_mde_pw_slot", None), getattr(yb, "_mde_pw_slot", None))
     return _SeBnCat.apply(ya, yb, bn_a.weight, bn_a.bias, pb_a, bn_b.weight, bn_b.bias, pb_b,
-                          w1, w2, meta(bn_a), meta(bn_b), stats_a, stats_b)
+                          w1, w2, meta(bn_a), meta(bn_b), stats_a, stats_b,
+                          slots if None not in slots else None)
 
 
 def pointwise_ok(conv: nn.Conv2d, x) -> bool:
@@ -1294,7 +1353,8 @@
 
     @staticmethod
     @_bn_fwd
-    def forward(ctx, r, d, weight, bias, gamma, beta, prebias, meta, stats, d_slot=None):
+    def forward(ctx, r, d, weight, bias, gamma, beta, prebias, meta, stats, d_slot=None,
+                pw_slot=None):
         dt = torch.bfloat16 if r.dtype == torch.bfloat16 else torch.float32
         r, d = r.to(dt).contiguous(), d.to(dt).contiguous()
         n, cin, h, w = r.shape
@@ -1323,6 +1383,7 @@
                   _abi.dtype_code(r), st)
         ctx.save_for_backward(r, d, wm, gamma, beta, scale, shift, mean, invstd)
         ctx.wshape, ctx.has_pb, ctx.d_slot = weight.shape, prebias is not None, d_slot
+        ctx.pw_slot = pw_slot if dt == torch.float32 else None
         return out
 
     @staticmethod
@@ -1342,10 +1403,18 @@
                   _abi.ptr(scale), _abi.ptr(shift), _abi.ptr(mean), _abi.ptr(wm), _abi.ptr(gs),
                   _abi.ptr(gw), _abi.ptr(gb), _abi.ptr(sums), n, cin, cout, h, w, _abi.ptr(ws),
                   _abi.dtype_code(gout), st)
-        gr = torch.empty_like(r)
         gg, gbeta = torch.empty_like(gamma), torch.empty_like(beta)
         gpb = torch.empty_like(gamma) if (ctx.has_pb and ctx.needs_input_grad[6]) else None
-        if sums is not None:
+        deferred = (ctx.pw_slot is not None and sums is not None and ctx.needs_input_grad[0]
+                    and gs.dtype == torch.float32)
+        gr = gs if deferred else torch.empty_like(r)
+        if deferred:
+            tab = torch.empty((5, cin), dtype=torch.float32, device=r.device)
+            _abi.call("mde_batchnorm_bwd_coef", _abi.ptr(gamma), _abi.ptr(beta), _abi.ptr(mean),
+                      _abi.ptr(invstd), 1, _abi.ptr(sums), _abi.ptr(tab), _abi.ptr(gg),
+                      _abi.ptr(gbeta), _abi.ptr(gpb), n, cin, h, w, st)
+            ctx.pw_slot.put(gs, 0, r, tab)
+        elif sums is not None:
             _abi.call("mde_batchnorm_bwd_apply", _abi.ptr(gs), _abi.ptr(r), None, _abi.ptr(gamma),
                       _abi.ptr(beta), _abi.ptr(mean), _abi.ptr(invstd), 1, _abi.ptr(sums),
                       _abi.ptr(gr), None, _abi.ptr(gg), _abi.ptr(gbeta), _abi.ptr(gpb), n, cin, h,
@@ -1361,7 +1430,7 @@
             gd = None
         else:
             gd = gs
-        return gr, gd, gw.view(ctx.wshape), gb, gg, gbeta, gpb, None, None, None
+        return gr, gd, gw.view(ctx.wshape), gb, gg, gbeta, gpb, None, None, None, None
 
 
 def skip_reduce_bn_ok(r, cout: int) -> bool:
@@ -1378,7 +1447,8 @@
     meta = (bn.running_mean if track else None, bn.running_var if track else None,
             bn.num_batches_tracked if track else None, bn.momentum, bn.eps)
     return _SkipReduceBN.apply(r, d, weight, bias, bn.weight, bn.bias, prebias, meta, stats,
-                               getattr(d, "_mde_grad_slot", None))
+                               getattr(d, "_mde_grad_slot", None),
+                               getattr(r, "_mde_pw_slot", None))
 
 
 class BatchNorm2d(nn.BatchNorm2d):
```

After: 1024 images/s (median of 6 runs). 2.2% higher.
